# xdsopl/dwt

Measured on AMD Instinct MI355X. Metric: Mpixels/s lossless encode+decode round-trip, higher is better.
Workload: dtype int32; 1 GPU; 4096x4096x1 8-bit synthetic smooth+noise frames, lossless, 128 frames per GPU per step (BASELINE.json configs[1] geometry); frames_per_gpu=128, parallelism=1 GPU

## Files before the change

### dwt_amd/csrc/unpack.hip

```cpp
#include "hilbert_dev.h"

#include <stdlib.h>
#include <string.h>
#include <vector>

namespace {

constexpr int TILE = 1024;
constexpr int MAX_PLANES = 16;
constexpr int MAX_SEGS = 3 * 16 * MAX_PLANES;
constexpr int CH_LOG2 = 7;
constexpr int CH_BITS = 1 << CH_LOG2;
constexpr int SCAN_BLOCK = 1024;
constexpr int LINK_ROUNDS = 12;
constexpr int FAM = 2;

struct UnpackGeom {
	int levels, C, W, H;
	long total;
	long lin_stride;
	int pixels[DWTX_MAX_LEVELS + 1];
	int tile_first[DWTX_MAX_LEVELS + 1];
	int levels_max;
	int *pyr;
	short *fine16;
	unsigned lv16;
	unsigned sq_levels;
	int side[DWTX_MAX_LEVELS + 1];
	const int *tile_base;
	const unsigned short *tile_cnt;
	const int *tile_blk;
};

struct DecInfo {
	int status;
	int W, H, C;
	int levels;
	int planes[3];
	int pmax;
	int level;
	int nsegs;
	int truncated;
	int missing[48];
	unsigned long long bits_used;
	unsigned hops, hopped_chunks;
	unsigned walked_tokens;
	unsigned zeros_left;
};

struct SegIndex {
	unsigned long long bit;
	unsigned long long sym_base;
	unsigned n1;
	unsigned cnt;
	unsigned desc;
	unsigned order;
};

struct SegResult {
	unsigned long long bit;
	unsigned order, cnt, ones;
	unsigned nhops, hopped, walked;
	unsigned ok;
	unsigned pad;
};

struct DWork {
	DecInfo *info;
	int *seg_desc;
	unsigned long long *seg_symbase;
	unsigned long long *seg_b2;
	unsigned *seg_n2done;
	int *segidx;
	int *nonsig;
	unsigned *symbits;
	unsigned short *tile_nonsig;
	unsigned *tile_rank;
	unsigned long long *count_base;
	long BW;
	int NT;
	unsigned short *exitX;
	unsigned short *entryE;
	unsigned long long *cs;
	unsigned *ct;
	unsigned *cg;
	unsigned long long *part_s;
	unsigned *part_t, *part_g;
	int *hop_seg;
	unsigned *hop_first, *hop_last, *hop_q0;
	unsigned *hop_entry;
	unsigned *hop_ntok;
	unsigned *breaks;
	unsigned *todo[2];
	unsigned *todo_count;
	long todo_round;
	long todo_cap;
	unsigned long long *dbg;
	int *nhops;
	int *nch;
	long NCH, NB;
	long MAX_HOPS;
	SegIndex *idx;
	SegResult *segres;
	int *idx_nsegs;
	unsigned *seg_slot;
	int fam;
	unsigned streak_max, scans_base;
};

__device__ __forceinline__ int vstream(const DWork &w, int row) { return (row / w.fam) * FAM + row % w.fam; }

__device__ __forceinline__ int popc_below(unsigned long long m)
{
	return __builtin_amdgcn_mbcnt_hi((unsigned)(m >> 32), __builtin_amdgcn_mbcnt_lo((unsigned)m, 0));
}


struct BitReader {
	const unsigned long long *w;
	long n64;
	unsigned long long end_bits;
	unsigned long long b;
	unsigned long long base;
	unsigned long long f0, f1, f2, f3, f4, f5;

	__device__ __forceinline__ unsigned long long ld(unsigned long long bit) const
	{
		const long i = (long)(bit >> 6);
		return i < n64 ? w[i] : 0ull;
	}
	__device__ void seek(unsigned long long nb)
	{
		b = nb;
		base = nb & ~63ull;
		f0 = ld(base);
		f1 = ld(base + 64);
		f2 = ld(base + 128);
		f3 = ld(base + 192);
		f4 = ld(base + 256);
		f5 = ld(base + 320);
	}
	__device__ __forceinline__ unsigned long long peek()
	{
		while (b - base >= 64) {
			f0 = f1;
			f1 = f2;
			f2 = f3;
			f3 = f4;
			f4 = f5;
			base += 64;
			f5 = ld(base + 320);
		}
		const int off = (int)(b - base);
		return off ? (f0 >> off) | (f1 << (64 - off)) : f0;
	}
	__device__ __forceinline__ unsigned long long avail() const { return end_bits > b ? end_bits - b : 0ull; }
	__device__ __forceinline__ bool read(int n, unsigned &v)
	{
		if ((unsigned long long)n > avail())
			return false;
		const unsigned long long win = peek();
		v = n >= 32 ? (unsigned)win : (unsigned)win & ((1u << n) - 1u);
		b += n;
		return true;
	}
	__device__ __forceinline__ bool vli(int &order, unsigned &val)
	{
		const unsigned long long win = peek();
		const unsigned long long av = avail();
		const int z = win ? __builtin_ctzll(win) : 64;
		if ((unsigned long long)z >= av)
			return false;
		const int top = order + z;
		if (top > 31)
			return false;
		const int need = z + 1 + top;
		if ((unsigned long long)need > av)
			return false;
		const unsigned rem = top ? (unsigned)(win >> (z + 1)) & (unsigned)((1ull << top) - 1ull) : 0u;
		val = rem + (1u << top) - (1u << order);
		order = top >= 2 ? top - 2 : 0;
		b += need;
		return true;
	}
	__device__ bool read_any(unsigned n, unsigned &v)
	{
		if (n <= 32u)
			return read((int)n, v);
		unsigned a = 0;
		for (unsigned i = 0; i < n; ++i) {
			unsigned bit;
			if (!read(1, bit))
				return false;
			a |= bit << (i & 31u);
		}
		v = a;
		return true;
	}
	__device__ int vli_any(int &order, unsigned &val)
	{
		if (vli(order, val))
			return 0;
		unsigned ord = (unsigned)order, sum = 0;
		for (;;) {
			if (avail() >= 64 && !peek()) {
				sum += 2u * 0xffffffffu;
				ord += 64;
				b += 64;
				continue;
			}
			unsigned bit;
			if (!read(1, bit))
				return 1;
			if (bit)
				break;
			sum += 1u << (ord & 31u);
			++ord;
		}
		unsigned a = 0;
		for (unsigned i = 0; i < ord; ++i) {
			unsigned bit;
			if (!read(1, bit))
				return 1;
			a |= bit << (i & 31u);
		}
		order = ord >= 2u ? (int)(ord - 2u) : 0;
		const int v = (int)(a + sum);
		if (v < 0)
			return 2;
		val = (unsigned)v;
		return 0;
	}
};

struct BitmapWriter {
	unsigned *sym;
	long cur;
	unsigned acc;
	bool lead;
	__device__ __forceinline__ void flush()
	{
		if (cur >= 0 && acc && lead)
			atomicOr(sym + cur, acc);
		acc = 0;
	}
	__device__ __forceinline__ void set_one(unsigned long long pos)
	{
		const long wi = (long)(pos >> 4);
		if (wi != cur) {
			flush();
			cur = wi;
		}
		acc |= 1u << ((pos & 15) * 2);
	}
	__device__ __forceinline__ void set_sign(unsigned long long pos) { acc |= 2u << ((pos & 15) * 2); }
};


struct ChunkWin {
	unsigned long long w0, w1, w2;
};

__device__ __forceinline__ ChunkWin chunk_load(const unsigned long long *w64, long n64, long chunk)
{
	ChunkWin c;
	const long i = chunk * (CH_BITS / 64);
	c.w0 = i < n64 ? w64[i] : 0ull;
	c.w1 = i + 1 < n64 ? w64[i + 1] : 0ull;
	c.w2 = i + 2 < n64 ? w64[i + 2] : 0ull;
	return c;
}

__device__ __forceinline__ unsigned long long chunk_win(const ChunkWin &c, int off)
{
	const int r = off & 63;
	const unsigned long long lo = off >> 6 ? c.w1 : c.w0, hi = off >> 6 ? c.w2 : c.w1;
	return r ? (lo >> r) | (hi << (64 - r)) : lo;
}

__device__ __forceinline__ unsigned bfm(unsigned width, unsigned offset)
{
	unsigned r;
	asm("v_bfm_b32 %0, %1, %2" : "=v"(r) : "v"(width), "v"(offset));
	return r;
}

__device__ __forceinline__ bool token_at(unsigned long long win, int o, int &len, unsigned &run, unsigned &neg, int &next)
{
	if (!win)
		return false;
	const int z = __builtin_ctzll(win);
	const int top = o + z;
	if (top > 31)
		return false;
	len = z + top + 2;
	run = (top ? (unsigned)(win >> (z + 1)) & (unsigned)((1ull << top) - 1ull) : 0u) + (1u << top) - (1u << o);
	neg = (unsigned)(win >> (z + 1 + top)) & 1u;
	next = top >= 2 ? top - 2 : 0;
	return true;
}

#pragma clang diagnostic ignored "-Wpass-failed"
template <class F>
__device__ __forceinline__ bool chunk_walk(const ChunkWin &c, int &off, int &o, F &&visit)
{
	const unsigned d[6] = { (unsigned)c.w0, (unsigned)(c.w0 >> 32), (unsigned)c.w1, (unsigned)(c.w1 >> 32),
		(unsigned)c.w2, (unsigned)(c.w2 >> 32) };
	bool dead = false, stop = false;
#pragma unroll
	for (int seg = 0; seg < CH_BITS / 32; ++seg) {
		for (;;) {
			const int bound = 32 * (seg + 1);
			bool fits = !(stop || dead), go = true;
			while (off < bound && fits && go) {
				const unsigned w32 = __builtin_amdgcn_alignbit(d[seg + 1], d[seg], (unsigned)off);
				const int z = __builtin_ctz(w32 | 0x80000000u);
				const int top = o + z;
				const int len = z + top + 2;
				fits = len <= 32;
				const unsigned run = __builtin_amdgcn_ubfe(w32, (unsigned)(z + 1), (unsigned)top) + bfm((unsigned)z, (unsigned)o);
				const unsigned neg = __builtin_amdgcn_ubfe(w32, (unsigned)(len - 1), 1u);
				go = visit(run, neg, fits);
				const bool adv = fits && go;
				off += adv ? len : 0;
				o = adv ? (int)__builtin_elementwise_sub_sat((unsigned)top, 2u) : o;
			}
			stop = stop || !go;
			const bool slow = !fits && !stop && !dead;
			if (!ballot64(slow))
				break;
			if (slow) {
				const int r = off & 31;
				const unsigned long long lo64 = d[seg] | ((unsigned long long)d[seg + 1] << 32);
				const unsigned long long w64 = r ? (lo64 >> r) | ((unsigned long long)d[seg + 2] << (64 - r)) : lo64;
				int len, next;
				unsigned run, neg;
				if (!token_at(w64, o, len, run, neg, next)) {
					dead = true;
				} else if (visit(run, neg, true)) {
					off += len;
					o = next;
				} else {
					stop = true;
				}
			}
		}
	}
	return !dead;
}

template <class V, class K, class U>
__device__ __forceinline__ bool chunk_walk_all(const ChunkWin &c, int &off, int &o, V &&visit, K &&keep, U &&undo)
{
	const unsigned d[6] = { (unsigned)c.w0, (unsigned)(c.w0 >> 32), (unsigned)c.w1, (unsigned)(c.w1 >> 32),
		(unsigned)c.w2, (unsigned)(c.w2 >> 32) };
	bool dead = false;
#pragma unroll
	for (int seg = 0; seg < CH_BITS / 32; ++seg) {
		for (;;) {
			const int bound = 32 * (seg + 1);
			int len = 0, o_prev = o;
			while (off < bound) {
				o_prev = o;
				keep();
				const unsigned w32 = __builtin_amdgcn_alignbit(d[seg + 1], d[seg], (unsigned)off);
				const int z = __builtin_ctz(w32 | 0x80000000u);
				const int top = o + z;
				len = z + top + 2;
				visit(__builtin_amdgcn_ubfe(w32, (unsigned)(z + 1), (unsigned)top) + bfm((unsigned)z, (unsigned)o),
					__builtin_amdgcn_ubfe(w32, (unsigned)(len - 1), 1u), len <= 32);
				off += len;
				o = (int)__builtin_elementwise_sub_sat((unsigned)top, 2u);
			}
			const bool slow = len > 32;
			if (!ballot64(slow))
				break;
			if (slow) {
				off -= len;
				o = o_prev;
				undo();
				const int r = off & 31;
				const unsigned long long lo64 = d[seg] | ((unsigned long long)d[seg + 1] << 32);
				const unsigned long long w64 = r ? (lo64 >> r) | ((unsigned long long)d[seg + 2] << (64 - r)) : lo64;
				int len64, next;
				unsigned run, neg;
				if (!token_at(w64, o, len64, run, neg, next)) {
					dead = true;
					off = 2 * CH_BITS + 64;
				} else {
					visit(run, neg, true);
					off += len64;
					o = next;
				}
			}
		}
	}
	return !dead;
}

__device__ __forceinline__ bool chunk_count(const ChunkWin &c, int &off, int &o, unsigned &tok, unsigned &sym)
{
	unsigned sym_prev = sym;
	return chunk_walk_all(c, off, o,
		[&](unsigned run, unsigned, bool) {
			sym = __builtin_elementwise_add_sat(sym, run + 1u);
			++tok;
		},
		[&]() { sym_prev = sym; },
		[&]() {
			--tok;
			sym = sym_prev;
		});
}

__device__ __forceinline__ unsigned wave_incl_add_u(unsigned v)
{
	v += (unsigned)__builtin_amdgcn_update_dpp(0, (int)v, 0x111, 0xf, 0xf, false);
	v += (unsigned)__builtin_amdgcn_update_dpp(0, (int)v, 0x112, 0xf, 0xf, false);
	v += (unsigned)__builtin_amdgcn_update_dpp(0, (int)v, 0x114, 0xf, 0xf, false);
	v += (unsigned)__builtin_amdgcn_update_dpp(0, (int)v, 0x118, 0xf, 0xf, false);
	v += (unsigned)__builtin_amdgcn_update_dpp(0, (int)v, 0x142, 0xa, 0xf, false);
	v += (unsigned)__builtin_amdgcn_update_dpp(0, (int)v, 0x143, 0xc, 0xf, false);
	return v;
}

struct ChunkScan {
	unsigned tok, sym;
	int off, o;
	unsigned cross_run;
	int cross_bits, cross_o;
};

__device__ __forceinline__ ChunkScan chunk_scan(const ChunkWin &c, int off, int o, unsigned need)
{
	const int lane = (int)threadIdx.x & 63;
	const unsigned d0 = (unsigned)c.w0, d1 = (unsigned)(c.w0 >> 32), d2 = (unsigned)c.w1, d3 = (unsigned)(c.w1 >> 32),
		d4 = (unsigned)c.w2;
	const bool up = lane >= 32;
	const unsigned winA = __builtin_amdgcn_alignbit(up ? d2 : d1, up ? d1 : d0, (unsigned)lane & 31u);
	const unsigned winB = __builtin_amdgcn_alignbit(up ? d4 : d3, up ? d3 : d2, (unsigned)lane & 31u);
	{
		const int zA = winA ? __builtin_ctz(winA) : 32, zB = winB ? __builtin_ctz(winB) : 32;
		int ordA = -1, ordB = -1, offf = __builtin_amdgcn_readfirstlane(off), of2 = __builtin_amdgcn_readfirstlane(o) + 2;
		while (offf < 64) {
			const int z = __builtin_amdgcn_readlane(zA, offf);
			ordA = lane == offf ? of2 : ordA;
			const int top2 = of2 + z;
			offf += top2 + z;
			of2 = max(top2 - 2, 2);
		}
		while (offf < 128) {
			const int z = __builtin_amdgcn_readlane(zB, offf - 64);
			ordB = lane == offf - 64 ? of2 : ordB;
			const int top2 = of2 + z;
			offf += top2 + z;
			of2 = max(top2 - 2, 2);
		}
		const int of = of2 - 2;
		ordA = ordA < 0 ? -1 : ordA - 2;
		ordB = ordB < 0 ? -1 : ordB - 2;
		const bool longA = ordA >= 0 && 2 * zA + ordA > 30, longB = ordB >= 0 && 2 * zB + ordB > 30;
		const int worst = ballot64(longA || longB) ? 31 : 0;
		if (worst <= 30) {
			constexpr unsigned CAP = 1u << 24;
			auto cost = [&](unsigned win, int z, int ord) -> unsigned {
				const int top = ord + z;
				const unsigned run = ((win >> ((z + 1) & 31)) & ((1u << (top & 31)) - 1u)) + (1u << (top & 31)) - (1u << (ord & 31));
				return ord < 0 ? 0u : min(run + 1u, CAP);
			};
			const unsigned cA = cost(winA, zA, ordA), cB = cost(winB, zB, ordB);
			const unsigned long long visA = ballot64(ordA >= 0), visB = ballot64(ordB >= 0);
			const bool capped = ballot64(cA == CAP || cB == CAP) != 0;
			int v = (int)(cA + cB);
			v += __builtin_amdgcn_update_dpp(0, v, 0xB1, 0xf, 0xf, true);
			v += __builtin_amdgcn_update_dpp(0, v, 0x4E, 0xf, 0xf, true);
			v += __builtin_amdgcn_update_dpp(0, v, 0x141, 0xf, 0xf, true);
			v += __builtin_amdgcn_update_dpp(0, v, 0x140, 0xf, 0xf, true);
			const unsigned symf = (unsigned)(__builtin_amdgcn_readlane(v, 0) + __builtin_amdgcn_readlane(v, 16) +
				__builtin_amdgcn_readlane(v, 32) + __builtin_amdgcn_readlane(v, 48));
			if (!capped && symf <= need) {
				ChunkScan r = { (unsigned)(__builtin_popcountll(visA) + __builtin_popcountll(visB)), symf, offf, of, 0u, 0, 0 };
				return r;
			}
			if (!capped) {
				const unsigned need_s = (unsigned)__builtin_amdgcn_readfirstlane((int)need);
				const unsigned pA = wave_incl_add_u(cA);
				const unsigned totA = (unsigned)__builtin_amdgcn_readlane((int)pA, 63);
				const unsigned pB = totA + wave_incl_add_u(cB);
				const unsigned long long fitA = ballot64(ordA >= 0 && pA <= need_s), fitB = ballot64(ordB >= 0 && pB <= need_s);
				const unsigned long long restA = visA & ~fitA, restB = visB & ~fitB;
				unsigned sym = 0;
				if (fitB)
					sym = (unsigned)__builtin_amdgcn_readlane((int)pB, 63 - __builtin_clzll(fitB));
				else if (fitA)
					sym = (unsigned)__builtin_amdgcn_readlane((int)pA, 63 - __builtin_clzll(fitA));
				int off2, o2, z2;
				unsigned c2;
				if (restA) {
					const int at = __builtin_ctzll(restA);
					off2 = at;
					o2 = __builtin_amdgcn_readlane(ordA, at);
					z2 = __builtin_amdgcn_readlane(zA, at);
					c2 = (unsigned)__builtin_amdgcn_readlane((int)cA, at);
				} else {
					const int at = __builtin_ctzll(restB);
					off2 = 64 + at;
					o2 = __builtin_amdgcn_readlane(ordB, at);
					z2 = __builtin_amdgcn_readlane(zB, at);
					c2 = (unsigned)__builtin_amdgcn_readlane((int)cB, at);
				}
				const int top2 = o2 + z2;
				ChunkScan r = { (unsigned)(__builtin_popcountll(fitA) + __builtin_popcountll(fitB)), sym, off2, o2, c2 - 1u, z2 + top2 + 1, max(top2, 2) - 2 };
				return r;
			}
		}
	}
	const unsigned need_s = (unsigned)__builtin_amdgcn_readfirstlane((int)need);
	unsigned tok = 0, left = need_s;
	off = __builtin_amdgcn_readfirstlane(off);
	o = __builtin_amdgcn_readfirstlane(o);
	auto token = [&](unsigned w32) -> bool {
		const int z = w32 ? __builtin_ctz(w32) : 32;
		const int top = o + z;
		const unsigned run = ((w32 >> ((z + 1) & 31)) & ((1u << (top & 31)) - 1u)) + (1u << (top & 31)) - (1u << o);
		const bool ok = z + top <= 30 && run < left;
		left -= ok ? run + 1u : 0u;
		tok += ok ? 1u : 0u;
		off += ok ? z + top + 2 : 0;
		o = ok ? max(top, 2) - 2 : o;
		return ok;
	};
	bool ok = true;
	while (ok && off < 64)
		ok = token((unsigned)__builtin_amdgcn_readlane((int)winA, off));
	while (ok && off < 128)
		ok = token((unsigned)__builtin_amdgcn_readlane((int)winB, off - 64));
	ChunkScan r = { tok, need_s - left, off, o, 0u, 0, 0 };
	return r;
}

constexpr int CHUNK_GRID = 2048;

constexpr int LINK_SHARDS = 64;
constexpr int LINK_RUN = 8;
constexpr int RUN_W = 2 * LINK_RUN + 2;

__device__ __forceinline__ bool link_parse(const DWork &w, const unsigned char *streams, long stream_stride, int vs, long ch)
{
	const int img = vs / FAM;
	const long ci = vs * (w.NCH + 1) + ch;
	const unsigned short in = w.exitX[vs * w.NCH + ch - 1];
	unsigned sym = 0, tok = 0;
	unsigned short out = 0xffff;
	if (in != 0xffff) {
		const ChunkWin c = chunk_load((const unsigned long long *)(streams + img * stream_stride), stream_stride >> 3, ch);
		int off = in & 0xff, o = in >> 8;
		if (chunk_count(c, off, o, tok, sym))
			out = (unsigned short)((off - CH_BITS) | (o << 8));
	}
	const unsigned short old = w.exitX[vs * w.NCH + ch];
	w.entryE[vs * w.NCH + ch] = in;
	w.cs[ci] = sym;
	w.ct[ci] = tok;
	w.exitX[vs * w.NCH + ch] = out;
	return out != old && ch + 1 < w.nch[img];
}

__device__ __forceinline__ void link_push(const DWork &w, int vs, long ch, bool want, unsigned *next_list, unsigned *next_count)
{
	const int lane = threadIdx.x & 63;
	const int shard = (int)((ch >> 8) % LINK_SHARDS);
	unsigned long long todo = ballot64(want);
	while (todo) {
		const int leader = __builtin_ctzll(todo);
		const int sh = __shfl(shard, leader);
		const unsigned long long same = ballot64(want && shard == sh) & todo;
		unsigned base = 0;
		if (lane == leader)
			base = atomicAdd(next_count + vs * LINK_SHARDS + sh, (unsigned)__builtin_popcountll(same));
		base = __shfl(base, leader);
		if (want && shard == sh)
			next_list[((long)vs * LINK_SHARDS + sh) * w.todo_cap + base +
				(unsigned)__builtin_popcountll(same & ((1ull << lane) - 1ull))] = (unsigned)ch;
		todo &= ~same;
	}
}

__device__ __forceinline__ unsigned link_state13(unsigned short s) { return s == 0xffff ? 0x1fffu : ((unsigned)s & 0x7fu) | ((unsigned)s >> 8) << 7; }
__device__ __forceinline__ unsigned short link_state16(unsigned s) { return s == 0x1fffu ? (unsigned short)0xffff : (unsigned short)((s & 0x7fu) | (s >> 7) << 8); }
__device__ __forceinline__ unsigned long long link_record(unsigned sym, unsigned tok, unsigned short in, unsigned short out)
{
	const unsigned long long s31 = sym < 0x7fffffffu ? sym : 0x7fffffffu;
	return s31 | (unsigned long long)tok << 31 | (unsigned long long)link_state13(in) << 38 | (unsigned long long)link_state13(out) << 51;
}


__global__ __launch_bounds__(256) __attribute__((amdgpu_num_sgpr(64), amdgpu_waves_per_eu(4))) void k_link_first(DWork w, const unsigned char *streams, long stream_stride)
{
	__shared__ unsigned long long words[256 * RUN_W + 4];
	__shared__ unsigned short sx[256];
	const int vs = vstream(w, blockIdx.y), img = vs / FAM;
	const long nch = w.nch[img];
	const unsigned short start = (unsigned short)((w.fam == 1 ? 0 : CH_BITS / 2) + vs % FAM);
	const unsigned long long *w64 = (const unsigned long long *)(streams + img * stream_stride);
	const long n64 = stream_stride >> 3;
	constexpr long SPAN = 256 * LINK_RUN;
	for (long base = (long)blockIdx.x * SPAN; base < nch; base += (long)gridDim.x * SPAN) {
		const long g0 = 2 * (base - 1);
#pragma unroll
		for (int k = 0; k < (2 * (int)SPAN + 3 + 255) / 256; ++k) {
			const int L = k * 256 + (int)threadIdx.x;
			const long gi = g0 + L;
			if (L < 2 * (int)SPAN + 3)
				words[L + (L / (2 * LINK_RUN)) * 2] = gi >= 0 && gi < n64 ? w64[gi] : 0ull;
		}
		__syncthreads();
		const long c0 = base + (long)threadIdx.x * LINK_RUN;
		unsigned long long *mine = words + threadIdx.x * RUN_W;
		auto word = [&](int i) { return mine[i + (i >= 2 * LINK_RUN ? 2 : 0)]; };
		unsigned short st = start, wexit = 0xffff;
		unsigned long long carry = word(0);
		for (int j = 0; j <= LINK_RUN; ++j) {
			const long chunk = c0 - 1 + j;
			ChunkWin c = { carry, word(2 * j + 1), word(2 * j + 2) };
			carry = c.w2;
			unsigned long long rec = ~0ull;
			if (chunk >= 0 && chunk < nch) {
				const unsigned short in = j == 0 || chunk == 0 || st == 0xffff ? start : st;
				int off = in & 0xff, o = in >> 8;
				unsigned sym = 0, tok = 0;
				const bool alive = chunk_count(c, off, o, tok, sym);
				st = alive ? (unsigned short)((off - CH_BITS) | (o << 8)) : (unsigned short)0xffff;
				rec = link_record(sym, tok, in, st);
			}
			if (j == 0)
				wexit = st;
			else
				mine[2 + j] = rec;
		}
		sx[threadIdx.x] = st;
		__syncthreads();
#pragma unroll
		for (int k = 0; k < LINK_RUN; ++k) {
			const int q = k * 256 + (int)threadIdx.x;
			const long chunk = base + q;
			const unsigned long long rec = words[(q / LINK_RUN) * RUN_W + 3 + q % LINK_RUN];
			if (rec != ~0ull) {
				if (chunk > 0) {
					w.entryE[vs * w.NCH + chunk] = link_state16((unsigned)(rec >> 38) & 0x1fffu);
					w.cs[vs * (w.NCH + 1) + chunk] = rec & 0x7fffffffull;
					w.ct[vs * (w.NCH + 1) + chunk] = (unsigned)(rec >> 31) & 0x7fu;
				}
				w.exitX[vs * w.NCH + chunk] = link_state16((unsigned)(rec >> 51));
			}
		}
		const bool redo = c0 > 0 && c0 < nch && (threadIdx.x == 0 || sx[threadIdx.x - 1] != wexit);
		link_push(w, vs, c0, redo, w.todo[1], w.todo_count + 2 * w.todo_round);
		__syncthreads();
	}
}

__global__ __launch_bounds__(256) __attribute__((amdgpu_num_sgpr(64))) void k_link_work(DWork w, const unsigned char *streams, long stream_stride, int cur, int round)
{
	const int vs = vstream(w, blockIdx.y), shard = blockIdx.x % LINK_SHARDS, part = blockIdx.x / LINK_SHARDS,
		parts = gridDim.x / LINK_SHARDS;
	const unsigned count = w.todo_count[round * w.todo_round + vs * LINK_SHARDS + shard];
	const unsigned *list = w.todo[cur] + ((long)vs * LINK_SHARDS + shard) * w.todo_cap;
	for (unsigned q0 = part * blockDim.x; q0 < count; q0 += parts * blockDim.x) {
		const unsigned q = q0 + threadIdx.x;
		bool moved = false;
		long ch = 0;
		if (q < count) {
			ch = list[q];
			moved = link_parse(w, streams, stream_stride, vs, ch);
		}
		link_push(w, vs, ch + 1, moved, w.todo[cur ^ 1], w.todo_count + (round + 1) * w.todo_round);
	}
}

struct Tri {
	unsigned long long s;
	unsigned t, g;
};

__device__ __forceinline__ Tri tri_add(Tri a, Tri b)
{
	Tri r = { a.s + b.s, a.t + b.t, a.g + b.g };
	return r;
}

__device__ __forceinline__ Tri tri_shfl_up(Tri v, int o)
{
	Tri r;
	r.s = __shfl_up(v.s, o);
	r.t = __shfl_up(v.t, o);
	r.g = __shfl_up(v.g, o);
	return r;
}

__device__ __forceinline__ Tri block_scan_tri(Tri v, Tri *wsum, Tri &total)
{
	const int lane = threadIdx.x & 63, wv = threadIdx.x >> 6;
	Tri inc = v;
	for (int o = 1; o < 64; o <<= 1) {
		const Tri t = tri_shfl_up(inc, o);
		if (lane >= o)
			inc = tri_add(inc, t);
	}
	if (lane == 63)
		wsum[wv] = inc;
	__syncthreads();
	Tri off = { 0, 0, 0 }, all = { 0, 0, 0 };
	for (int k = 0; k < 4; ++k) {
		if (k < wv)
			off = tri_add(off, wsum[k]);
		all = tri_add(all, wsum[k]);
	}
	__syncthreads();
	total = all;
	Tri ex = { off.s + inc.s - v.s, off.t + inc.t - v.t, off.g + inc.g - v.g };
	return ex;
}

struct Quad {
	ulonglong2 s01, s23;
	uint4 t, g;
};

__device__ __forceinline__ Quad quad_load(const DWork &w, long at)
{
	Quad q;
	q.s01 = *reinterpret_cast<const ulonglong2 *>(w.cs + at);
	q.s23 = *reinterpret_cast<const ulonglong2 *>(w.cs + at + 2);
	q.t = *reinterpret_cast<const uint4 *>(w.ct + at);
	q.g = *reinterpret_cast<const uint4 *>(w.cg + at);
	return q;
}

__device__ __forceinline__ void quad_store(const DWork &w, long at, const Quad &q)
{
	*reinterpret_cast<ulonglong2 *>(w.cs + at) = q.s01;
	*reinterpret_cast<ulonglong2 *>(w.cs + at + 2) = q.s23;
	*reinterpret_cast<uint4 *>(w.ct + at) = q.t;
	*reinterpret_cast<uint4 *>(w.cg + at) = q.g;
}

constexpr int SCAN_GRID = 1024;

__global__ __launch_bounds__(256) void k_scan_local(DWork w)
{
	__shared__ Tri wsum[4];
	const int vs = vstream(w, blockIdx.y);
	const long n = w.NCH + 1, nch = w.nch[vs / FAM], used = nch + 1;
	unsigned short *exitX = w.exitX + (long)vs * w.NCH, *entryE = w.entryE + (long)vs * w.NCH;
	for (long vb = blockIdx.x; vb * SCAN_BLOCK < used; vb += gridDim.x) {
		const long i = vb * SCAN_BLOCK + 4 * threadIdx.x;
		const bool in = i < used;
		Quad q;
		q.s01 = q.s23 = make_ulonglong2(0ull, 0ull);
		q.t = q.g = make_uint4(0u, 0u, 0u, 0u);
		if (in) {
			q = quad_load(w, vs * n + i);
			unsigned long long *sv[4] = { &q.s01.x, &q.s01.y, &q.s23.x, &q.s23.y };
			unsigned *tv[4] = { &q.t.x, &q.t.y, &q.t.z, &q.t.w }, *gv[4] = { &q.g.x, &q.g.y, &q.g.z, &q.g.w };
			unsigned short prev = i >= 1 && i - 1 < nch ? exitX[i - 1] : (unsigned short)0xffff;
#pragma unroll
			for (int e = 0; e < 4; ++e) {
				const long c = i + e;
				unsigned flag;
				if (c == 0 || c >= nch) {
					flag = c == 0 ? 1u : 0u;
					*sv[e] = 0;
					*tv[e] = 0;
				} else {
					const unsigned short x = exitX[c];
					const bool bad = prev == 0xffff || entryE[c] != prev || x == 0xffff;
					flag = bad ? 1u : 0u;
					if (bad) {
						*sv[e] = 0;
						*tv[e] = 0;
					}
					prev = x;
				}
				if (c == 0)
					prev = nch > 0 ? exitX[0] : (unsigned short)0xffff;
				*gv[e] = flag;
				if (c < nch)
					entryE[c] = (unsigned short)flag;
			}
		}
		const Tri mine = { q.s01.x + q.s01.y + q.s23.x + q.s23.y, q.t.x + q.t.y + q.t.z + q.t.w, q.g.x + q.g.y + q.g.z + q.g.w };
		Tri total;
		const Tri pre = block_scan_tri(mine, wsum, total);
		if (in) {
			Quad o;
			o.s01.x = pre.s;
			o.s01.y = o.s01.x + q.s01.x;
			o.s23.x = o.s01.y + q.s01.y;
			o.s23.y = o.s23.x + q.s23.x;
			o.t.x = pre.t;
			o.t.y = o.t.x + q.t.x;
			o.t.z = o.t.y + q.t.y;
			o.t.w = o.t.z + q.t.z;
			o.g.x = pre.g;
			o.g.y = o.g.x + q.g.x;
			o.g.z = o.g.y + q.g.y;
			o.g.w = o.g.z + q.g.z;
			quad_store(w, vs * n + i, o);
		}
		if (threadIdx.x == 0) {
			w.part_s[vs * w.NB + vb] = total.s;
			w.part_t[vs * w.NB + vb] = total.t;
			w.part_g[vs * w.NB + vb] = total.g;
		}
		__syncthreads();
	}
}

__global__ __launch_bounds__(256) void k_scan_parts(DWork w)
{
	__shared__ Tri wsum[4];
	const int img = vstream(w, blockIdx.x);
	const long nb = (w.nch[img / FAM] + 1 + SCAN_BLOCK - 1) / SCAN_BLOCK;
	Tri carry = { 0, 0, 0 };
	for (long b0 = 0; b0 < nb; b0 += 256) {
		const long i = b0 + threadIdx.x;
		Tri v = { 0, 0, 0 };
		if (i < nb) {
			v.s = w.part_s[img * w.NB + i];
			v.t = w.part_t[img * w.NB + i];
			v.g = w.part_g[img * w.NB + i];
		}
		Tri total;
		const Tri pre = block_scan_tri(v, wsum, total);
		if (i < nb) {
			w.part_s[img * w.NB + i] = carry.s + pre.s;
			w.part_t[img * w.NB + i] = carry.t + pre.t;
			w.part_g[img * w.NB + i] = carry.g + pre.g;
		}
		carry = tri_add(carry, total);
	}
}

__global__ __launch_bounds__(256) void k_scan_add(DWork w)
{
	const int vs = vstream(w, blockIdx.y);
	const long n = w.NCH + 1, nch = w.nch[vs / FAM], used = nch + 1;
	const unsigned short *flags = w.entryE + (long)vs * w.NCH;
	unsigned *breaks = w.breaks + (long)vs * w.NCH;
	for (long vb = blockIdx.x; vb * SCAN_BLOCK < used; vb += gridDim.x) {
		const long i = vb * SCAN_BLOCK + 4 * threadIdx.x;
		if (i >= used)
			continue;
		const unsigned long long ps = w.part_s[vs * w.NB + vb];
		const unsigned pt = w.part_t[vs * w.NB + vb], pg = w.part_g[vs * w.NB + vb];
		Quad q = quad_load(w, vs * n + i);
		q.s01.x += ps;
		q.s01.y += ps;
		q.s23.x += ps;
		q.s23.y += ps;
		q.t.x += pt;
		q.t.y += pt;
		q.t.z += pt;
		q.t.w += pt;
		q.g.x += pg;
		q.g.y += pg;
		q.g.z += pg;
		q.g.w += pg;
		if (vb)
			quad_store(w, vs * n + i, q);
		const unsigned g4[4] = { q.g.x, q.g.y, q.g.z, q.g.w };
#pragma unroll
		for (int e = 0; e < 4; ++e)
			if (i + e < nch && flags[i + e])
				breaks[g4[e]] = (unsigned)(i + e);
	}
}

__global__ __launch_bounds__(256) __attribute__((amdgpu_waves_per_eu(8))) void k_hopbits(DWork w, const unsigned char *streams, long stream_stride)
{
	constexpr int HB_WORDS = 16;
	constexpr int HB_WIN = 2048;
	__shared__ unsigned hb[256 * (HB_WORDS + 1)];
	static_assert(HB_WIN <= 256 * (HB_WORDS + 1), "the workgroup's window lies inside the per-thread rows");
	unsigned *win = hb;
	__shared__ unsigned win_last;
	for (int i = 0; i <= HB_WORDS; ++i)
		hb[threadIdx.x * (HB_WORDS + 1) + i] = 0u;
	const int img = blockIdx.y;
	const int nh = w.nhops[img];
	const long nchunks = w.nch[img];
	const unsigned *hf = w.hop_first + (long)img * w.MAX_HOPS, *hl = w.hop_last + (long)img * w.MAX_HOPS;
	for (long vblock = blockIdx.x; vblock * blockDim.x < nchunks; vblock += gridDim.x) {
	const long chunk = vblock * blockDim.x + threadIdx.x;
	const unsigned first_chunk = (unsigned)(vblock * blockDim.x);
	int lo = 0, hi = nh;
	while (lo < hi) {
		const int mid = (lo + hi) >> 1;
		if (hl[mid] < first_chunk)
			lo = mid + 1;
		else
			hi = mid;
	}
	unsigned *sym = w.symbits + img * w.BW;
	const long n = w.NCH + 1;
	ChunkWin c;
	bool loaded = false;
	unsigned *mybuf = hb + threadIdx.x * (HB_WORDS + 1);
	auto piece = [&](int h) {
		const int hs = w.hop_seg[(long)img * w.MAX_HOPS + h];
		const int k = hs & 0xffff, vs = img * FAM + (hs >> 16);
		if ((w.seg_desc[(long)img * MAX_SEGS + k] >> 8) == 0)
			return;
		if (!loaded) {
			c = chunk_load((const unsigned long long *)(streams + img * stream_stride), stream_stride >> 3, chunk);
			loaded = true;
		}
		unsigned long long pos = w.seg_symbase[(long)img * MAX_SEGS + k] + w.hop_q0[(long)img * w.MAX_HOPS + h];
		const unsigned entry = w.hop_entry[(long)img * w.MAX_HOPS + h];
		unsigned left = w.hop_ntok[(long)img * w.MAX_HOPS + h];
		int off, o;
		if (entry == 0xffffffffu) {
			pos += w.cs[vs * n + chunk] - w.cs[vs * n + hf[h]];
			const unsigned short in = w.exitX[vs * w.NCH + chunk - 1];
			off = in & 0xff;
			o = in >> 8;
		} else {
			off = (int)(entry & 0xff);
			o = (int)(entry >> 8);
		}
		unsigned *wp = sym + (pos >> 4);
		const unsigned rp0 = (unsigned)(pos & 15);
		unsigned rp = rp0;
		bool beyond = false;
		const int off0 = off, o0 = o;
		chunk_walk(c, off, o, [&](unsigned run, unsigned neg, bool counts) {
			const bool take = counts && left != 0u;
			rp += take ? run : 0u;
			const unsigned wi = rp >> 4;
			beyond = beyond || (take && wi >= (unsigned)HB_WORDS);
			atomicOr(&mybuf[wi < (unsigned)HB_WORDS ? wi : (unsigned)HB_WORDS], take ? (1u | (neg << 1)) << ((rp & 15u) * 2u) : 0u);
			rp += take ? 1u : 0u;
			left -= take ? 1u : 0u;
			return left != 0u || !counts;
		});
		if (beyond) {
			unsigned rq = rp0, lq = w.hop_ntok[(long)img * w.MAX_HOPS + h];
			int off1 = off0, o1 = o0;
			chunk_walk(c, off1, o1, [&](unsigned run, unsigned neg, bool counts) {
				const bool take = counts && lq != 0u;
				rq += take ? run : 0u;
				if (take && (rq >> 4) >= (unsigned)HB_WORDS)
					atomicOr(wp + (rq >> 4), (1u | (neg << 1)) << ((rq & 15u) * 2u));
				rq += take ? 1u : 0u;
				lq -= take ? 1u : 0u;
				return lq != 0u || !counts;
			});
			mybuf[HB_WORDS] = 0u;
		}
		const unsigned lastw = rp > rp0 ? (rp - 1) >> 4 : 0u;
#pragma unroll
		for (int i = 0; i < HB_WORDS; ++i) {
			const unsigned v = mybuf[i];
			if (v) {
				if (i == 0 || (unsigned)i >= lastw)
					atomicOr(wp + i, v);
				else
					wp[i] = v;
				mybuf[i] = 0u;
			}
		}
	};
	const bool mine = chunk < w.nch[img] && chunk >= 1;
	if (lo < nh && hf[lo] <= first_chunk && hl[lo] >= first_chunk + blockDim.x - 1 && (lo + 1 >= nh || hf[lo + 1] > first_chunk + blockDim.x - 1)) {
		const int hs = w.hop_seg[(long)img * w.MAX_HOPS + lo];
		const int k = hs & 0xffff, vs = img * FAM + (hs >> 16);
		const bool stitched = w.hop_entry[(long)img * w.MAX_HOPS + lo] == 0xffffffffu && first_chunk >= 1;
		if (!stitched) {
			if (mine)
				piece(lo);
			continue;
		}
		if ((w.seg_desc[(long)img * MAX_SEGS + k] >> 8) == 0)
			continue;
		const unsigned long long seg0 = w.seg_symbase[(long)img * MAX_SEGS + k] + w.hop_q0[(long)img * w.MAX_HOPS + lo] -
			w.cs[vs * n + hf[lo]];
		const unsigned long long base_w = (seg0 + w.cs[vs * n + first_chunk]) >> 4;
		if (threadIdx.x == 0)
			win_last = 0u;
		__syncthreads();
		{
			const ChunkWin cw = chunk_load((const unsigned long long *)(streams + img * stream_stride), stream_stride >> 3, chunk);
			const unsigned short in = w.exitX[vs * w.NCH + chunk - 1];
			int off = in & 0xff, o = in >> 8;
			unsigned roff = (unsigned)(seg0 + w.cs[vs * n + chunk] - (base_w << 4));
			const unsigned roff0 = roff;
			unsigned *gp = sym + base_w;
			unsigned roff_prev = roff;
			chunk_walk_all(cw, off, o,
				[&](unsigned run, unsigned neg, bool fits) {
					roff += run;
					const unsigned wi = roff >> 4;
					const unsigned bits = fits ? (1u | (neg << 1)) << ((roff & 15u) * 2u) : 0u;
					if (wi < (unsigned)HB_WIN)
						atomicOr(&win[wi], bits);
					else if (fits)
						atomicOr(gp + wi, bits);
					++roff;
				},
				[&]() { roff_prev = roff; }, [&]() { roff = roff_prev; });
			if (roff > roff0) {
				const unsigned lw = (roff - 1) >> 4;
				atomicMax(&win_last, lw < (unsigned)HB_WIN - 1u ? lw : (unsigned)HB_WIN - 1u);
			}
		}
		__syncthreads();
		{
			const unsigned lastw = win_last;
			unsigned *gp = sym + base_w;
			for (unsigned i = threadIdx.x; i <= lastw; i += 256) {
				const unsigned v = win[i];
				win[i] = 0u;
				if (i > 0 && i < lastw)
					gp[i] = v;
				else if (v)
					atomicOr(gp + i, v);
			}
		}
		__syncthreads();
		continue;
	}
	if (!mine)
		continue;
	int h = lo;
	while (h < nh && hl[h] < (unsigned)chunk)
		++h;
	for (; h < nh && hf[h] <= (unsigned)chunk; ++h)
		piece(h);
	}
}

__global__ __launch_bounds__(256) void k_part_reset(DWork h, int cnt)
{
	const long t = (long)blockIdx.x * blockDim.x + threadIdx.x;
	const long per_round = (long)cnt * FAM * LINK_SHARDS;
	if (t < per_round)
		for (int r = 0; r < LINK_ROUNDS + 2; ++r)
			h.todo_count[r * h.todo_round + t] = 0u;
	if (t < cnt)
		h.nhops[t] = 0;
	if (t < (long)cnt * 48 * MAX_PLANES)
		h.segidx[t] = 0;
	if (t < (long)cnt * (long)(sizeof(DecInfo) / sizeof(int)))
		reinterpret_cast<int *>(h.info)[t] = 0;
}

__device__ int read_preamble(BitReader &br, const UnpackGeom &g, const unsigned char *s8, unsigned long long len, long stream_stride,
	int &order, int (&planes)[3], int *root, long root_stride)
{
	if (len < 6 || s8[0] != 'W' || s8[1] != (g.C == 3 ? '6' : '5') ||
		(s8[2] | (s8[3] << 8)) + 1 != g.W || (s8[4] | (s8[5] << 8)) + 1 != g.H)
		return 1;
	br.w = (const unsigned long long *)s8;
	br.n64 = stream_stride >> 3;
	br.end_bits = len * 8;
	br.seek(48);
	order = 0;
	for (int c = 0; c < g.C; ++c) {
		unsigned cnt;
		if (br.vli_any(order, cnt))
			return 1;
		if (cnt)
			for (int i = 0; i < g.pixels[0]; ++i) {
				unsigned v, neg = 0;
				if (!br.read_any(cnt, v))
					return 1;
				if (v && !br.read(1, neg))
					return 1;
				if (root)
					root[c * root_stride + i] = neg ? -(int)v : (int)v;
			}
	}
	for (int c = 0; c < g.C; ++c) {
		unsigned p;
		if (br.vli_any(order, p))
			return 1;
		if (p > MAX_PLANES)
			return 2;
		planes[c] = (int)p;
	}
	return 0;
}

__global__ __launch_bounds__(64) void k_peek(UnpackGeom g, const unsigned char *streams, long stream_stride, const unsigned long long *lens,
	long BW, unsigned *clear_words, int n)
{
	const int img = blockIdx.x * blockDim.x + threadIdx.x;
	if (img >= n)
		return;
	const unsigned char *s8 = streams + img * stream_stride;
	const unsigned long long len = lens[img] < (unsigned long long)stream_stride ? lens[img] : (unsigned long long)stream_stride;
	BitReader br;
	int order, planes[3] = { 0, 0, 0 };
	unsigned long long words = 0;
	if (!read_preamble(br, g, s8, len, stream_stride, order, planes, nullptr, 0)) {
		unsigned long long per = 0;
		for (int l = 0; l < g.levels; ++l)
			per += ((unsigned long long)(g.pixels[l + 1] - g.pixels[l]) + 31) & ~31ull;
		unsigned long long sym = ((unsigned long long)(g.pixels[1] - g.pixels[0]) + 31) & ~31ull;
		for (int c = 0; c < g.C; ++c)
			sym += (unsigned long long)planes[c] * per;
		words = ((sym >> 4) + 128 + 3) & ~3ull;
	}
	clear_words[img] = (unsigned)(words < (unsigned long long)BW ? words : (unsigned long long)BW);
}

__global__ __launch_bounds__(256) void k_clear_bitmaps(unsigned *bits, long BW, const unsigned *clear_words)
{
	uint4 *dst = reinterpret_cast<uint4 *>(bits + (long)blockIdx.y * BW);
	const unsigned quads = clear_words[blockIdx.y] >> 2;
	for (unsigned i = blockIdx.x * blockDim.x + threadIdx.x; i < quads; i += gridDim.x * blockDim.x)
		dst[i] = make_uint4(0u, 0u, 0u, 0u);
}


template <class F, class M>
__device__ __forceinline__ bool walk_schedule(const UnpackGeom &g, const int (&planes)[3], int pmax, int &level, M &&one_less_missing, F &&seg)
{
	const int levels = g.levels;
	const int layers_max = 2 * (levels > pmax ? levels : pmax) - 1;
	bool stop = g.levels_max == 0;
	if (!stop && pmax == planes[0]) {
		level = 0;
		if (seg(0, 0, planes[0] - 1))
			one_less_missing(0);
		else
			stop = true;
	}
	for (int layer = 0; !stop && layer < layers_max; ++layer) {
		for (int l = 0; !stop && l < levels && l <= layer + 1; ++l) {
			if (l >= g.levels_max) {
				stop = true;
				break;
			}
			const int p = pmax - 1 - (layer + 1 - l);
			if (p < 0 || p >= planes[0])
				continue;
			level = level < l ? l : level;
			if (seg(0, l, p))
				one_less_missing(l);
			else
				stop = true;
		}
		for (int l = 0; !stop && l < levels && l <= layer; ++l) {
			if (l >= g.levels_max) {
				stop = true;
				break;
			}
			const int p = pmax - 1 - (layer - l);
			for (int c = 1; !stop && c < g.C; ++c) {
				if (p < 0 || p >= planes[c])
					continue;
				level = level < l ? l : level;
				if (seg(c, l, p))
					one_less_missing(c * 16 + l);
				else
					stop = true;
			}
		}
	}
	return stop;
}

constexpr unsigned WALK_STREAK_MAX = 256u, WALK_SCANS_BASE = 256u;
constexpr unsigned WALK_GAVE_UP = 0xffffffffu;

__device__ __forceinline__ void info_begin(DecInfo &I, const UnpackGeom &g)
{
	I.status = 1;
	I.W = g.W;
	I.H = g.H;
	I.C = g.C;
	I.levels = g.levels;
	I.level = -1;
	I.nsegs = 0;
	I.truncated = 0;
	I.pmax = 0;
	for (int i = 0; i < 48; ++i)
		I.missing[i] = 0;
}

template <bool SEG>
__global__ __launch_bounds__(64) void k_tokenize(UnpackGeom g, DWork w, const unsigned char *streams, long stream_stride,
	const unsigned long long *lens, int *lin, int n)
{
	const int img = SEG ? blockIdx.y : blockIdx.x;
	if (img >= n)
		return;
	const int seg_k = SEG ? (int)blockIdx.x : 0;
	if (SEG && seg_k >= w.idx_nsegs[img])
		return;
	DecInfo &I = w.info[img];
	const unsigned char *s8 = streams + img * stream_stride;
	const unsigned long long len = lens[img] < (unsigned long long)stream_stride ? lens[img] : (unsigned long long)stream_stride;
	BitReader br;
	int order = 0;
	int planes[3] = { 0, 0, 0 };
	int pmax = 0;
	int nonsig_own[1] = { 0 };
	int nonsig_v = 0;
	SegIndex *idx = w.idx + (long)img * MAX_SEGS;
	if (!SEG) {
		info_begin(I, g);
		if (const int bad = read_preamble(br, g, s8, len, stream_stride, order, planes, lin + (long)img * g.C * g.lin_stride, g.lin_stride)) {
			I.status = bad;
			return;
		}
		for (int c = 0; c < g.C; ++c) {
			I.planes[c] = planes[c];
			pmax = planes[c] > pmax ? planes[c] : pmax;
		}
		I.pmax = pmax;
		I.status = 0;
		for (int c = 0; c < g.C; ++c)
			for (int l = 0; l < g.levels; ++l)
				I.missing[c * 16 + l] = planes[c];
		{
			const int lv = (int)threadIdx.x & 15, ch = (int)threadIdx.x >> 4;
			nonsig_v = ch < g.C && lv < g.levels ? g.pixels[lv + 1] - g.pixels[lv] : 0;
		}
	} else {
		br.w = (const unsigned long long *)s8;
		br.n64 = stream_stride >> 3;
		br.end_bits = len * 8;
		br.b = idx[seg_k].bit < br.end_bits ? idx[seg_k].bit : br.end_bits;
		br.base = 0;
		br.f0 = br.f1 = br.f2 = br.f3 = br.f4 = br.f5 = 0;
		order = (int)(idx[seg_k].order & 31u);
		nonsig_own[0] = (int)idx[seg_k].n1;
	}
	int *sd = w.seg_desc + (long)img * MAX_SEGS;
	unsigned long long *ssym = w.seg_symbase + (long)img * MAX_SEGS;
	unsigned long long *sb2 = w.seg_b2 + (long)img * MAX_SEGS;
	unsigned *sn2 = w.seg_n2done + (long)img * MAX_SEGS;
	int *sidx = w.segidx + (long)img * 3 * 16 * MAX_PLANES;
	BitmapWriter bm;
	bm.sym = w.symbits + img * w.BW;
	bm.cur = -1;
	bm.acc = 0;
	bm.lead = threadIdx.x == 0;
	const int wl = (int)threadIdx.x;

	unsigned cnt = SEG ? idx[seg_k].cnt : 0u;
	unsigned long long symtotal = SEG ? idx[seg_k].sym_base : 0ull;
	int nsegs = seg_k, level = -1;

	const unsigned short *exitX0 = w.exitX + (long)img * FAM * w.NCH;
	const unsigned long long *CS0 = w.cs + (long)img * FAM * (w.NCH + 1);
	const unsigned *CT0 = w.ct + (long)img * FAM * (w.NCH + 1), *CG0 = w.cg + (long)img * FAM * (w.NCH + 1);
	const unsigned *BR0 = w.breaks + (long)img * FAM * w.NCH;
	const unsigned long long *s64 = (const unsigned long long *)s8;
	const long lastsafe = br.end_bits >= 64 + CH_BITS ? (long)((br.end_bits - 64) >> CH_LOG2) - 1 : -1;
#ifdef DWTX_DEBUG_HOOKS
	unsigned long long t_hop = 0, t_fast = 0, t_load = 0, t_scan = 0, t_care = 0, n_care = 0, t_all0 = __builtin_readcyclecounter(), t_mark = 0;
#define WALK_MARK() t_mark = __builtin_readcyclecounter()
#define WALK_ADD(acc) do { const unsigned long long t_now = __builtin_readcyclecounter(); acc += t_now - t_mark; t_mark = t_now; } while (0)
#else
#define WALK_MARK()
#define WALK_ADD(acc)
#endif
	unsigned scans = 0, streak = 0;
	bool giveup = false;
	long checked = -1;
	int nhops = 0;
	unsigned hopped = 0, walked = 0;
	bool br_synced = !SEG;
	bool eof = false;
	const long hop0 = (long)img * w.MAX_HOPS + (SEG ? (long)w.seg_slot[(long)img * (MAX_SEGS + 1) + seg_k] : 0l);
	const long hop_cap = SEG ? (long)(w.seg_slot[(long)img * (MAX_SEGS + 1) + seg_k + 1] - w.seg_slot[(long)img * (MAX_SEGS + 1) + seg_k]) : w.MAX_HOPS;
	int *hop_seg = w.hop_seg + hop0;
	unsigned *hop_first = w.hop_first + hop0, *hop_last = w.hop_last + hop0, *hop_q0 = w.hop_q0 + hop0, *hop_entry = w.hop_entry + hop0,
		*hop_ntok = w.hop_ntok + hop0;

	auto segment = [&](int c, int l, int p) -> bool {
		const int num = g.pixels[l + 1] - g.pixels[l];
		const int n1 = p < 0 ? num : SEG ? nonsig_own[0] : __builtin_amdgcn_readlane(nonsig_v, c * 16 + l);
		const int n2 = num - n1;
		const int k = nsegs++;
		const unsigned long long sym0 = symtotal;
		if (!SEG) {
			SegIndex e;
			e.bit = br.b;
			e.sym_base = sym0;
			e.n1 = (unsigned)n1;
			e.cnt = cnt;
			e.desc = (unsigned)(c | (l << 4) | ((p + 1) << 8));
			e.order = (unsigned)order;
			idx[k] = e;
		}
		symtotal += ((unsigned long long)num + 31) & ~31ull;
		sd[k] = c | (l << 4) | ((p + 1) << 8);
		ssym[k] = sym0;
		sb2[k] = 0;
		sn2[k] = 0;
		if (p >= 0)
			sidx[(c * 16 + l) * MAX_PLANES + p] = k + 1;
		int q = 0, ones = 0;
		bool ok = true;
		streak = 0;
		while (q < n1) {
			unsigned zr;
			if (cnt == 0) {
				const long ci = (long)(br.b >> CH_LOG2);
				if (ci >= 1 && ci <= lastsafe && nhops < hop_cap) {
					const unsigned need = (unsigned)(n1 - q);
					const int rel = (int)(br.b - ((unsigned long long)ci << CH_LOG2));
					bool moved = false;
					WALK_MARK();
					if (ci != checked) {
						checked = ci;
						for (int fam = 0; fam < w.fam && !moved; ++fam) {
							const unsigned ep = exitX0[fam * w.NCH + ci - 1];
							if (ep == 0xffffu || (int)(ep & 0xffu) != rel || (int)(ep >> 8) != order)
								continue;
							const unsigned long long *CS = CS0 + fam * (w.NCH + 1);
							const unsigned *CT = CT0 + fam * (w.NCH + 1), *CG = CG0 + fam * (w.NCH + 1);
							const unsigned g0 = CG[ci], g1 = CG[ci + 1], gtot = CG[w.nch[img]];
							if (g1 != g0)
								continue;
							const unsigned long long s0 = CS[ci];
							long hi = g0 < gtot ? (long)BR0[fam * w.NCH + g0] - 1 : lastsafe;
							hi = hi < lastsafe ? hi : lastsafe;
							long lo = ci - 1;
							if (hi >= ci && CS[hi + 1] - s0 <= (unsigned long long)need) {
								lo = hi;
							} else {
								hi = hi - 1;
								while (lo < hi) {
									const long span = hi - lo, stride = (span + 63) >> 6;
									const long step = (long)(wl + 1) * stride;
									const long probe = lo + (step < span ? step : span);
									const int t = __builtin_popcountll(ballot64(CS[probe + 1] - s0 <= (unsigned long long)need));
									const long reach = (long)t * stride, next = (long)(t + 1) * stride;
									hi = t == 64 ? hi : lo + (next < span ? next : span) - 1;
									lo = lo + (reach < span ? reach : span);
								}
							}
							if (lo >= ci) {
								hop_seg[nhops] = k | (fam << 16);
								hop_first[nhops] = (unsigned)ci;
								hop_last[nhops] = (unsigned)lo;
								hop_q0[nhops] = (unsigned)q;
								hop_entry[nhops] = 0xffffffffu;
								hop_ntok[nhops] = 0xffffffffu;
								++nhops;
								hopped += (unsigned)(lo - ci + 1);
								q += (int)(CS[lo + 1] - s0);
								ones += (int)(CT[lo + 1] - CT[ci]);
								const unsigned eq = exitX0[fam * w.NCH + lo];
								order = (int)(eq >> 8);
								br.b = ((unsigned long long)(lo + 1) << CH_LOG2) + (eq & 0xffu);
								br_synced = false;
								moved = true;
							}
						}
					}
					WALK_ADD(t_hop);
					if (moved)
						streak = 0;
					if (!moved) {
						++scans;
						++streak;
						if (w.fam < FAM && (streak > w.streak_max || scans > w.scans_base + 16u * (unsigned)nsegs + (unsigned)(lastsafe >> 9))) {
							giveup = true;
							return false;
						}
						const ChunkWin cwv = chunk_load(s64, br.n64, ci);
#ifdef DWTX_DEBUG_HOOKS
						asm volatile("s_waitcnt vmcnt(0) lgkmcnt(0)" ::: "memory");
						WALK_ADD(t_load);
#endif
						const ChunkScan cs = chunk_scan(cwv, rel, order, need);
#ifdef DWTX_DEBUG_HOOKS
						WALK_ADD(t_scan);
#endif
						const unsigned tok = cs.tok, sym = cs.sym;
						const int off = cs.off, o = cs.o;
						if (tok) {
							hop_seg[nhops] = k;
							hop_first[nhops] = (unsigned)ci;
							hop_last[nhops] = (unsigned)ci;
							hop_q0[nhops] = (unsigned)q;
							hop_entry[nhops] = (unsigned)rel | ((unsigned)order << 8);
							hop_ntok[nhops] = tok;
							++nhops;
							walked += tok;
							q += (int)sym;
							ones += (int)tok;
							order = o;
							br.b = ((unsigned long long)ci << CH_LOG2) + (unsigned)off;
							br_synced = false;
							moved = true;
						}
						if (cs.cross_bits && q < n1) {
							const unsigned rem = (unsigned)(n1 - q);
							++walked;
							order = cs.cross_o;
							br.b = ((unsigned long long)ci << CH_LOG2) + (unsigned)off + (unsigned)cs.cross_bits;
							br_synced = false;
							q = n1;
							cnt = cs.cross_run - rem + 1;
							WALK_ADD(t_fast);
							break;
						}
					}
					WALK_ADD(t_fast);
					if (moved)
						continue;
				}
#ifdef DWTX_DEBUG_HOOKS
				WALK_MARK();
				++n_care;
#endif
				if (!br_synced) {
					br.seek(br.b);
					br_synced = true;
				}
				unsigned v;
				const int bad = br.vli_any(order, v);
				if (bad) {
					ok = false;
					eof = bad == 1;
					break;
				}
				++walked;
				zr = v;
#ifdef DWTX_DEBUG_HOOKS
				WALK_ADD(t_care);
#endif
			} else {
				zr = cnt - 1;
			}
			const unsigned rem = (unsigned)(n1 - q);
			if (zr >= rem) {
				q = n1;
				cnt = zr - rem + 1;
				break;
			}
			q += (int)zr;
			cnt = 0;
			if (p >= 0)
				bm.set_one(sym0 + (unsigned)q);
			++ones;
			if (!br_synced) {
				br.seek(br.b);
				br_synced = true;
			}
			unsigned neg;
			if (!br.read(1, neg)) {
				++q;
				ok = false;
				eof = true;
				break;
			}
			if (neg && p >= 0)
				bm.set_sign(sym0 + (unsigned)q);
			++q;
		}
		if (p >= 0) {
			if (SEG)
				nonsig_own[0] = n1 - ones;
			else
				nonsig_v = wl == c * 16 + l ? n1 - ones : nonsig_v;
		}
		if (!ok)
			return false;
		if (p >= 0 && n2 > 0) {
			if (cnt > 0) {
				if (cnt != 1) {
					--cnt;
					return false;
				}
				cnt = 0;
			}
			sb2[k] = br.b;
			const unsigned long long av = br.avail();
			if ((unsigned long long)n2 > av) {
				sn2[k] = (unsigned)av;
				br.b = br.end_bits;
				eof = true;
				return false;
			}
			sn2[k] = (unsigned)n2;
			br.b += (unsigned)n2;
			br_synced = false;
		}
		return true;
	};

	bool stop = false;
	if (SEG) {
		const unsigned d = idx[seg_k].desc;
		const int c = (int)(d & 15u), l = (int)((d >> 4) & 15u), p = (int)(d >> 8) - 1;
		const unsigned long long ring = (unsigned long long)(g.pixels[l < g.levels ? l + 1 : 1] - g.pixels[l < g.levels ? l : 0]);
		const unsigned long long sym_cap = (unsigned long long)w.BW * 16ull;
		const bool sane = c < g.C && l < g.levels && p < MAX_PLANES && (unsigned long long)idx[seg_k].n1 <= ring && idx[seg_k].order <= 31u &&
			ring + 32ull <= sym_cap && idx[seg_k].sym_base <= sym_cap - ring - 32ull;
		const bool went = sane && segment(c, l, p);
		bm.flush();
		SegResult r;
		r.bit = br.b;
		r.order = (unsigned)order;
		r.cnt = cnt;
		r.ones = sane ? idx[seg_k].n1 - (unsigned)nonsig_own[0] : 0u;
		r.nhops = (unsigned)nhops;
		r.hopped = hopped;
		r.walked = walked;
		r.ok = went && !giveup && !eof ? 1u : 0u;
		r.pad = 0u;
		w.segres[(long)img * MAX_SEGS + seg_k] = r;
		return;
	}
	int missing_v = wl < 48 && (wl >> 4) < g.C && (wl & 15) < g.levels ? planes[wl >> 4 < 3 ? wl >> 4 : 0] : 0;
	stop = walk_schedule(g, planes, pmax, level, [&](int i) { missing_v = wl == i ? missing_v - 1 : missing_v; }, segment);
	if (wl < 48 && (wl >> 4) < g.C && (wl & 15) < g.levels)
		I.missing[wl] = missing_v;
	bm.flush();
	if (giveup) {
		w.nhops[img] = 0;
		I.hops = WALK_GAVE_UP;
		return;
	}
	w.nhops[img] = nhops;
	I.hops = (unsigned)nhops;
	I.hopped_chunks = hopped;
	I.walked_tokens = walked;
	I.zeros_left = cnt;
#ifdef DWTX_DEBUG_HOOKS
	if (w.dbg) { w.dbg[img * 8 + 0] = __builtin_readcyclecounter() - t_all0; w.dbg[img * 8 + 1] = t_hop; w.dbg[img * 8 + 2] = t_fast; w.dbg[img * 8 + 3] = scans;
		w.dbg[img * 8 + 4] = t_load; w.dbg[img * 8 + 5] = t_scan; w.dbg[img * 8 + 6] = t_care; w.dbg[img * 8 + 7] = n_care; }
#endif
	I.level = level;
	I.nsegs = nsegs;
	I.truncated = stop ? (eof ? 3 : 1) : 0;
	I.bits_used = br.b;
}

__global__ __launch_bounds__(64) void k_segprep(DWork w, const unsigned long long *lens, long stream_stride, int n)
{
	const int img = blockIdx.x * blockDim.x + threadIdx.x;
	if (img >= n)
		return;
	const int K = w.idx_nsegs[img];
	const SegIndex *idx = w.idx + (long)img * MAX_SEGS;
	unsigned *slot = w.seg_slot + (long)img * (MAX_SEGS + 1);
	const unsigned long long end_bits = 8ull * (lens[img] < (unsigned long long)stream_stride ? lens[img] : (unsigned long long)stream_stride);
	bool good = K > 0 && K <= MAX_SEGS;
	unsigned long long at = 0;
	for (int k = 0; good && k < K; ++k) {
		const unsigned long long b = idx[k].bit, nb = k + 1 < K ? idx[k + 1].bit : end_bits;
		good = b <= nb && nb <= end_bits && idx[k].sym_base < (unsigned long long)w.BW * 16ull && idx[k].order <= 31u;
		slot[k] = (unsigned)at;
		at += 8ull + ((nb - b) >> (CH_LOG2 + 3));
	}
	slot[K > 0 && K <= MAX_SEGS ? K : 0] = (unsigned)at;
	if (!good || at > (unsigned long long)w.MAX_HOPS)
		w.idx_nsegs[img] = 0;
}

__global__ __launch_bounds__(64) void k_segjoin(UnpackGeom g, DWork w, const unsigned char *streams, long stream_stride,
	const unsigned long long *lens, int *lin, int n)
{
	const int img = blockIdx.x;
	if (img >= n)
		return;
	const int lane = threadIdx.x;
	DecInfo &I = w.info[img];
	info_begin(I, g);
	const unsigned char *s8 = streams + img * stream_stride;
	const unsigned long long len = lens[img] < (unsigned long long)stream_stride ? lens[img] : (unsigned long long)stream_stride;
	BitReader br;
	int order = 0, planes[3] = { 0, 0, 0 };
	if (const int bad = read_preamble(br, g, s8, len, stream_stride, order, planes, lin + (long)img * g.C * g.lin_stride, g.lin_stride)) {
		I.status = bad;
		return;
	}
	int pmax = 0;
	for (int c = 0; c < g.C; ++c) {
		I.planes[c] = planes[c];
		pmax = planes[c] > pmax ? planes[c] : pmax;
	}
	I.pmax = pmax;
	I.status = 0;
	for (int c = 0; c < g.C; ++c)
		for (int l = 0; l < g.levels; ++l)
			I.missing[c * 16 + l] = planes[c];
	const int K = w.idx_nsegs[img];
	const SegIndex *idx = w.idx + (long)img * MAX_SEGS;
	const SegResult *res = w.segres + (long)img * MAX_SEGS;
	int nonsig[48];
	for (int c = 0; c < g.C; ++c)
		for (int l = 0; l < g.levels; ++l)
			nonsig[c * 16 + l] = g.pixels[l + 1] - g.pixels[l];
	unsigned long long at = br.b, symtotal = 0;
	unsigned cnt = 0, hopped = 0, walked = 0;
	int k = 0, level = -1;
	bool good = K > 0 && g.levels_max >= g.levels;
	const bool stop = walk_schedule(g, planes, pmax, level, [&](int i) { --I.missing[i]; }, [&](int c, int l, int p) {
		const int num = g.pixels[l + 1] - g.pixels[l];
		const int n1 = p < 0 ? num : nonsig[c * 16 + l];
		good = good && k < K;
		if (good) {
			const SegIndex e = idx[k];
			const SegResult r = res[k];
			good = e.desc == (unsigned)(c | (l << 4) | ((p + 1) << 8)) && e.bit == at && e.order == (unsigned)order && e.cnt == cnt &&
				e.n1 == (unsigned)n1 && e.sym_base == symtotal && r.ok != 0u && r.ones <= (unsigned)n1;
			if (good) {
				at = r.bit;
				order = (int)r.order;
				cnt = r.cnt;
				if (p >= 0)
					nonsig[c * 16 + l] = n1 - (int)r.ones;
				symtotal += ((unsigned long long)num + 31) & ~31ull;
				hopped += r.hopped;
				walked += r.walked;
				++k;
			}
		}
		return good;
	});
	good = good && !stop && k == K;
	if (!good) {
		w.nhops[img] = 0;
		I.hops = WALK_GAVE_UP;
		return;
	}
	const unsigned *slot = w.seg_slot + (long)img * (MAX_SEGS + 1);
	const long h0 = (long)img * w.MAX_HOPS;
	unsigned total = 0;
	for (int j = 0; j < K; ++j) {
		const unsigned nh = res[j].nhops, from = slot[j];
		if (from != total)
			for (unsigned i0 = 0; i0 < nh; i0 += 64) {
				const unsigned i = i0 + (unsigned)lane;
				int a = 0;
				unsigned b = 0, c2 = 0, d = 0, e = 0, f = 0;
				if (i < nh) {
					a = w.hop_seg[h0 + from + i];
					b = w.hop_first[h0 + from + i];
					c2 = w.hop_last[h0 + from + i];
					d = w.hop_q0[h0 + from + i];
					e = w.hop_entry[h0 + from + i];
					f = w.hop_ntok[h0 + from + i];
				}
				if (i < nh) {
					w.hop_seg[h0 + total + i] = a;
					w.hop_first[h0 + total + i] = b;
					w.hop_last[h0 + total + i] = c2;
					w.hop_q0[h0 + total + i] = d;
					w.hop_entry[h0 + total + i] = e;
					w.hop_ntok[h0 + total + i] = f;
				}
			}
		total += nh;
	}
	w.nhops[img] = (int)total;
	I.hops = total;
	I.hopped_chunks = hopped;
	I.walked_tokens = walked;
	I.zeros_left = cnt;
	I.level = level;
	I.nsegs = K;
	I.truncated = 0;
	I.bits_used = at;
}


__global__ __launch_bounds__(1024) void k_rank(UnpackGeom g, DWork w, int p)
{
	__shared__ unsigned wsum[16];
	__shared__ unsigned carry;
	const int l = blockIdx.x;
	const int plane = blockIdx.y;
	const int img = plane / g.C, c = plane - img * g.C;
	const int k1 = w.info[img].status ? 0 : w.segidx[((long)img * 48 + c * 16 + l) * MAX_PLANES + p];
	if (threadIdx.x == 0)
		w.count_base[(long)plane * 16 + l] = k1 ? 1ull + 2ull * w.seg_symbase[(long)img * MAX_SEGS + k1 - 1] : 0ull;
	if (!k1)
		return;
	const int t0 = g.tile_first[l], nt = g.tile_first[l + 1] - t0;
	const unsigned short *ns = w.tile_nonsig + (long)plane * w.NT + t0;
	unsigned *rank = w.tile_rank + ((long)plane * MAX_PLANES + p) * w.NT + t0;
	const int lane = threadIdx.x & 63, wv = threadIdx.x >> 6;
	if (threadIdx.x == 0)
		carry = 0;
	__syncthreads();
	for (int b0 = 0; b0 < nt; b0 += 1024) {
		const int i = b0 + threadIdx.x;
		const unsigned v = i < nt ? ns[i] : 0u;
		unsigned inc = v;
		for (int o = 1; o < 64; o <<= 1) {
			const unsigned t = __shfl_up(inc, o);
			if (lane >= o)
				inc += t;
		}
		if (lane == 63)
			wsum[wv] = inc;
		__syncthreads();
		unsigned woff = 0, all = 0;
		for (int k = 0; k < 16; ++k) {
			const unsigned s = wsum[k];
			woff += k < wv ? s : 0u;
			all += s;
		}
		const unsigned cy = carry;
		if (i < nt)
			rank[i] = cy + woff + inc - v;
		__syncthreads();
		if (threadIdx.x == 0)
			carry = cy + all;
		__syncthreads();
	}
}

__global__ __launch_bounds__(256) void k_count(UnpackGeom g, DWork w, int p)
{
	const int tile = blockIdx.x * blockDim.x + threadIdx.x;
	const int plane = blockIdx.y;
	const int img = plane / g.C;
	if (tile >= w.NT)
		return;
	int l = 0;
	while (l + 1 < g.levels && tile >= g.tile_first[l + 1])
		++l;
	const unsigned long long cb = w.count_base[(long)plane * 16 + l];
	if (!cb)
		return;
	unsigned short *ns = w.tile_nonsig + (long)plane * w.NT + tile;
	unsigned *rk = w.tile_rank + ((long)plane * MAX_PLANES + p) * w.NT + tile;
	const unsigned n = *ns;
	if (!n)
		return;
	const unsigned *sym = w.symbits + img * w.BW;
	const unsigned long long a = cb - 1ull + 2ull * *rk;
	const unsigned long long e = a + 2ull * n;
	const long first = (long)(a >> 5), last = (long)((e - 1) >> 5);
	unsigned ones = 0;
#pragma unroll 4
	for (long w0 = first & ~3l; w0 <= last; w0 += 4) {
		const uint4 v = *reinterpret_cast<const uint4 *>(sym + w0);
		const unsigned x[4] = { v.x, v.y, v.z, v.w };
#pragma unroll
		for (int q = 0; q < 4; ++q) {
			const long wi = w0 + q;
			unsigned m = x[q] & 0x55555555u;
			if (wi < first || wi > last)
				m = 0u;
			if (wi == first)
				m &= ~0u << (a & 31);
			if (wi == last && (e & 31))
				m &= (1u << (e & 31)) - 1u;
			ones += (unsigned)__builtin_popcount(m);
		}
	}
	if (ones) {
		*ns = (unsigned short)(n - ones);
		*rk |= 0x80000000u;
	}
}

__device__ __forceinline__ void bit_transpose8(unsigned &lo, unsigned &hi)
{
	unsigned t;
	t = (lo ^ (lo >> 7)) & 0x00AA00AAu;
	lo ^= t ^ (t << 7);
	t = (hi ^ (hi >> 7)) & 0x00AA00AAu;
	hi ^= t ^ (t << 7);
	t = (lo ^ (lo >> 14)) & 0x0000CCCCu;
	lo ^= t ^ (t << 14);
	t = (hi ^ (hi >> 14)) & 0x0000CCCCu;
	hi ^= t ^ (t << 14);
	const unsigned nlo = (lo & 0x0F0F0F0Fu) | ((hi << 4) & 0xF0F0F0F0u);
	hi = ((lo >> 4) & 0x0F0F0F0Fu) | (hi & 0xF0F0F0F0u);
	lo = nlo;
}

struct DepositTables {
	unsigned char sym[16 * 256];
	unsigned char ref[16 * 16];
};

constexpr DepositTables make_deposit_tables()
{
	DepositTables t{};
	for (unsigned m = 0; m < 16; ++m) {
		for (unsigned s = 0; s < 256; ++s) {
			unsigned ones = 0, signs = 0, k = 0;
			for (unsigned j = 0; j < 4; ++j)
				if ((m >> j) & 1u) {
					const unsigned one = (s >> (2 * k)) & 1u, sg = (s >> (2 * k + 1)) & 1u;
					ones |= one << j;
					signs |= (one & sg) << j;
					++k;
				}
			t.sym[m * 256 + s] = (unsigned char)(ones | signs << 4);
		}
		for (unsigned b = 0; b < 16; ++b) {
			unsigned out = 0, k = 0;
			for (unsigned j = 0; j < 4; ++j)
				if ((m >> j) & 1u) {
					out |= ((b >> k) & 1u) << j;
					++k;
				}
			t.ref[m * 16 + b] = (unsigned char)out;
		}
	}
	return t;
}

__device__ const DepositTables DEPOSIT = make_deposit_tables();

struct __attribute__((packed, aligned(4))) Int4S {
	int x, y, z, w;
};

__global__ __launch_bounds__(256) __attribute__((amdgpu_waves_per_eu(6))) void k_apply_all(UnpackGeom g, DWork w, const unsigned char *streams, long stream_stride, int *lin)
{
	__shared__ __attribute__((aligned(16))) unsigned char dep[sizeof(DepositTables)];
	static_assert(sizeof(DepositTables) == 17 * 256, "one 16-byte piece and one byte per thread");
	*reinterpret_cast<uint4 *>(dep + 16 * threadIdx.x) = *reinterpret_cast<const uint4 *>(DEPOSIT.sym + 16 * threadIdx.x);
	dep[4096 + threadIdx.x] = DEPOSIT.ref[threadIdx.x];
	__syncthreads();
	const unsigned char *dsym = dep, *dref = dep + 4096;
	const int lane = threadIdx.x & 63;
	const int tile = blockIdx.x * 4 + (threadIdx.x >> 6);
	const int plane = blockIdx.y;
	if (tile >= w.NT)
		return;
	const int img = plane / g.C, c = plane - img * g.C;
	const DecInfo &I = w.info[img];
	if (I.status)
		return;
	int l = 0;
	while (l + 1 < g.levels && tile >= g.tile_first[l + 1])
		++l;
	const unsigned tbase = (unsigned)g.tile_base[tile];
	const long base = g.pixels[l] + (long)tbase;
	const int nvalid = g.tile_cnt[tile];
	const int first = 16 * lane;
	const int nv = nvalid - first < 0 ? 0 : nvalid - first > 16 ? 16 : nvalid - first;
	const int vb = first < nvalid ? first : nvalid;
	const unsigned *sym = w.symbits + img * w.BW;
	const unsigned *stream = (const unsigned *)(streams + img * stream_stride);
	const long stream_words = stream_stride >> 2;
	unsigned R[8] = { 0u, 0u, 0u, 0u, 0u, 0u, 0u, 0u };
	int p_last = 0, rows_in = 0;
	auto push_row = [&](unsigned row16) {
		if (rows_in >= 8) {
#pragma unroll
			for (int k = 7; k >= 4; --k)
				R[k] = __builtin_amdgcn_alignbit(R[k], R[k - 1], 16);
		}
		if (rows_in >= 6)
			R[3] = __builtin_amdgcn_alignbit(R[3], R[2], 16);
		if (rows_in >= 4)
			R[2] = __builtin_amdgcn_alignbit(R[2], R[1], 16);
		if (rows_in >= 2)
			R[1] = __builtin_amdgcn_alignbit(R[1], R[0], 16);
		R[0] = (R[0] << 16) | row16;
		++rows_in;
	};
	unsigned neg = 0;
	const unsigned valid16 = nv >= 16 ? 0xffffu : (1u << nv) - 1u;
	unsigned ins = valid16;

	constexpr int AP_BATCH = 8, SYMW = 66, REFW = 34;
	static_assert(AP_BATCH * (SYMW + REFW) <= SQ_WORDS, "the plane slices share the wave's square staging area");
	__shared__ __attribute__((aligned(16))) unsigned ap_mem[4][SQ_WORDS];
	unsigned (*ap_sym)[SYMW] = reinterpret_cast<unsigned (*)[SYMW]>(ap_mem[threadIdx.x >> 6]);
	unsigned (*ap_ref)[REFW] = reinterpret_cast<unsigned (*)[REFW]>(ap_mem[threadIdx.x >> 6] + AP_BATCH * SYMW);
	__shared__ unsigned ap_rank[4][MAX_PLANES], ap_n2[4][MAX_PLANES], ap_refbit[4][MAX_PLANES];
	const int wv = threadIdx.x >> 6;
	unsigned my_tr = 0, my_n2 = 0;
	unsigned long long my_sb = 0, my_b2 = 0;
	bool my_live = false;
	if (lane < MAX_PLANES && lane < I.planes[c]) {
		const int k1 = w.segidx[((long)img * 48 + c * 16 + l) * MAX_PLANES + lane];
		if (k1) {
			my_live = true;
			my_tr = w.tile_rank[((long)plane * MAX_PLANES + lane) * w.NT + tile];
			my_sb = w.seg_symbase[(long)img * MAX_SEGS + k1 - 1];
			my_b2 = w.seg_b2[(long)img * MAX_SEGS + k1 - 1];
			my_n2 = w.seg_n2done[(long)img * MAX_SEGS + k1 - 1];
		}
	}
	const unsigned long long livem = ballot64(my_live), flagm = ballot64(my_live && (my_tr >> 31));
	const int ptop = flagm ? 63 - __builtin_clzll(flagm) : -1;
	unsigned long long todo = ptop >= 0 ? livem & ((2ull << ptop) - 1ull) : 0ull;
	while (todo) {
		int pl[AP_BATCH];
		unsigned long long t2 = todo;
#pragma unroll
		for (int q = 0; q < AP_BATCH; ++q) {
			pl[q] = t2 ? 63 - __builtin_clzll(t2) : -1;
			t2 &= pl[q] >= 0 ? ~(1ull << pl[q]) : ~0ull;
		}
		unsigned sv0[AP_BATCH], sv1[AP_BATCH], rv[AP_BATCH];
#pragma unroll
		for (int q = 0; q < AP_BATCH; ++q) {
			sv0[q] = sv1[q] = rv[q] = 0u;
			if (pl[q] < 0)
				continue;
			const unsigned rank = (unsigned)__builtin_amdgcn_readlane((int)my_tr, pl[q]) & 0x7fffffffu;
			const unsigned long long sb = ((unsigned long long)(unsigned)__builtin_amdgcn_readlane((int)(my_sb >> 32), pl[q]) << 32) |
				(unsigned)__builtin_amdgcn_readlane((int)my_sb, pl[q]);
			const unsigned long long b2 = ((unsigned long long)(unsigned)__builtin_amdgcn_readlane((int)(my_b2 >> 32), pl[q]) << 32) |
				(unsigned)__builtin_amdgcn_readlane((int)my_b2, pl[q]);
			const unsigned n2 = (unsigned)__builtin_amdgcn_readlane((int)my_n2, pl[q]);
			const unsigned *sp = sym + (sb >> 4) + (rank >> 4);
			sv0[q] = sp[lane];
			if (lane < SYMW - 64)
				sv1[q] = sp[64 + lane];
			const unsigned r2t = tbase - rank;
			const unsigned long long rbit = b2 + r2t;
			const long rw = (long)(rbit >> 5) + lane;
			if (lane < REFW && r2t < n2 && rw < stream_words)
				rv[q] = stream[rw];
			if (lane == 0) {
				ap_rank[wv][pl[q]] = rank;
				ap_n2[wv][pl[q]] = n2;
				ap_refbit[wv][pl[q]] = (unsigned)(rbit & 31);
			}
		}
#pragma unroll
		for (int q = 0; q < AP_BATCH; ++q) {
			if (pl[q] < 0)
				continue;
			ap_sym[q][lane] = sv0[q];
			if (lane < SYMW - 64)
				ap_sym[q][64 + lane] = sv1[q];
			if (lane < REFW)
				ap_ref[q][lane] = rv[q];
		}
		sq_wave_sync();
		const int nbatch = __builtin_popcountll(todo) < AP_BATCH ? __builtin_popcountll(todo) : AP_BATCH;
#pragma unroll 1
		for (int q = 0; q < nbatch; ++q) {
			const int p = 63 - __builtin_clzll(todo);
			todo &= ~(1ull << p);
			const unsigned rank = ap_rank[wv][p], n2done = ap_n2[wv][p];
			const unsigned ci = (unsigned)__builtin_popcount(ins);
			const unsigned nb = wave_incl_add_u(ci) - ci;
			const unsigned srel = (rank & 15u) + nb;
			const unsigned *sw = ap_sym[q] + (srel >> 4);
			unsigned s32 = __builtin_amdgcn_alignbit(sw[1], sw[0], (srel & 15u) * 2u);
			const unsigned sb4 = (unsigned)vb - nb;
			const unsigned r2 = tbase - rank + sb4;
			const unsigned cs = (unsigned)nv - ci;
			const unsigned avail = r2 < n2done ? (n2done - r2 < cs ? n2done - r2 : cs) : 0u;
			const unsigned rrel = ap_refbit[wv][p] + sb4;
			const unsigned *rwp = ap_ref[q] + (rrel >> 5);
			unsigned r16 = __builtin_amdgcn_alignbit(rwp[1], rwp[0], rrel & 31u) & bfm(avail, 0u);
			const unsigned sig = valid16 & ~ins;
			unsigned ones16 = 0, sgn16 = 0, ref16 = 0;
#pragma unroll
			for (int n4 = 0; n4 < 4; ++n4) {
				const unsigned mi = (ins >> (4 * n4)) & 15u, ms = (sig >> (4 * n4)) & 15u;
				const unsigned es = dsym[mi * 256u + (s32 & 255u)], er = dref[ms * 16u + (r16 & 15u)];
				ones16 |= (es & 15u) << (4 * n4);
				sgn16 |= (es >> 4) << (4 * n4);
				ref16 |= er << (4 * n4);
				s32 >>= 2 * __builtin_popcount(mi);
				r16 >>= __builtin_popcount(ms);
			}
			const unsigned bits16 = ones16 | ref16;
			neg |= sgn16;
			ins &= ~ones16;
			for (int gap = rows_in ? p_last - p - 1 : 0; gap > 0; --gap)
				push_row(0u);
			push_row(bits16);
			p_last = p;
		}
		sq_wave_sync();
	}
	unsigned mag[16];
	{
		unsigned lo[2], hi[2];
#pragma unroll
		for (int gg = 0; gg < 2; ++gg) {
			const unsigned sel = (unsigned)gg * 0x01010101u + 0x06040200u;
			lo[gg] = __builtin_amdgcn_perm(R[1], R[0], sel);
			hi[gg] = __builtin_amdgcn_perm(R[3], R[2], sel);
			bit_transpose8(lo[gg], hi[gg]);
		}
#pragma unroll
		for (int i = 0; i < 16; ++i)
			mag[i] = __builtin_amdgcn_ubfe((i & 4) ? hi[i >> 3] : lo[i >> 3], 8u * (i & 3), 8u);
		if (rows_in > 8) {
#pragma unroll
			for (int gg = 0; gg < 2; ++gg) {
				const unsigned sel = (unsigned)gg * 0x01010101u + 0x06040200u;
				lo[gg] = __builtin_amdgcn_perm(R[5], R[4], sel);
				hi[gg] = __builtin_amdgcn_perm(R[7], R[6], sel);
				bit_transpose8(lo[gg], hi[gg]);
			}
#pragma unroll
			for (int i = 0; i < 16; ++i)
				mag[i] |= __builtin_amdgcn_ubfe((i & 4) ? hi[i >> 3] : lo[i >> 3], 8u * (i & 3), 8u) << 8;
		}
#pragma unroll
		for (int i = 0; i < 16; ++i)
			mag[i] <<= p_last;
	}
	if (((g.sq_levels >> l) & 1u) && nvalid == TILE) {
		const int m = I.missing[c * 16 + l] - 2;
		const int bias = m >= 0 ? 1 << m : 0;
		int val[16];
#pragma unroll
		for (int i = 0; i < 16; ++i) {
			int v = ((neg >> i) & 1u) ? -(int)mag[i] : (int)mag[i];
			if (bias && v)
				v += v < 0 ? -bias : bias;
			val[i] = v;
		}
		if ((g.lv16 >> l) & 1u)
			store_square16(g.fine16 + (long)plane * g.lin_stride, g.W, g.side[l], g.tile_blk[tile], lane, ap_mem[threadIdx.x >> 6], val);
		else
			store_square16(g.pyr + (long)plane * g.lin_stride, g.W, g.side[l], g.tile_blk[tile], lane, ap_mem[threadIdx.x >> 6], val);
		return;
	}
	int *dst = lin + (long)plane * g.lin_stride + base + first;
	if (nvalid == TILE) {
#pragma unroll
		for (int q = 0; q < 4; ++q) {
			Int4S v;
			v.x = ((neg >> (4 * q)) & 1u) ? -(int)mag[4 * q] : (int)mag[4 * q];
			v.y = ((neg >> (4 * q + 1)) & 1u) ? -(int)mag[4 * q + 1] : (int)mag[4 * q + 1];
			v.z = ((neg >> (4 * q + 2)) & 1u) ? -(int)mag[4 * q + 2] : (int)mag[4 * q + 2];
			v.w = ((neg >> (4 * q + 3)) & 1u) ? -(int)mag[4 * q + 3] : (int)mag[4 * q + 3];
			*reinterpret_cast<Int4S *>(dst + 4 * q) = v;
		}
	} else {
#pragma unroll
		for (int i = 0; i < 16; ++i)
			if (i < nv)
				dst[i] = ((neg >> i) & 1u) ? -(int)mag[i] : (int)mag[i];
	}
}

__global__ __launch_bounds__(256) void k_tiles_init(UnpackGeom g, DWork w, int nplanes)
{
	const int tile = blockIdx.x * blockDim.x + threadIdx.x;
	const int plane = blockIdx.y;
	if (tile >= w.NT || plane >= nplanes)
		return;
	int l = 0;
	while (l + 1 < g.levels && tile >= g.tile_first[l + 1])
		++l;
	w.tile_nonsig[(long)plane * w.NT + tile] = g.tile_cnt[tile];
}

__global__ __launch_bounds__(256) void k_nch(DWork w, const unsigned long long *lens, int n)
{
	const int i = blockIdx.x * blockDim.x + threadIdx.x;
	if (i >= n)
		return;
	const unsigned long long bits = lens[i] * 8ull;
	long c = (long)((bits + CH_BITS - 1) / CH_BITS);
	c = (c + 1 + 3) / 4 * 4 - 1;
	w.nch[i] = (int)(c < w.NCH ? c : w.NCH);
}

}

template <class F> static void dwork_tables(DWork &w, unsigned *&clear_words, int C, F &&f)
{
	auto t = [&](int slot, auto *&table, long elems) { f(slot, table, elems, 1l); };
	t(SLOT_UP_SMALL, w.info, 1);
	t(SLOT_UP_SMALL, w.segidx, 48 * MAX_PLANES);
	t(SLOT_UP_SMALL, w.seg_desc, MAX_SEGS);
	t(SLOT_UP_SMALL, w.seg_symbase, MAX_SEGS);
	t(SLOT_UP_SMALL, w.seg_b2, MAX_SEGS);
	t(SLOT_UP_SMALL, w.seg_n2done, MAX_SEGS);
	t(SLOT_UP_SMALL, w.nonsig, 48);
	t(SLOT_UP_BITS, w.symbits, w.BW);
	t(SLOT_UP_TILES, w.tile_nonsig, (long)C * w.NT);
	t(SLOT_UP_TILES, w.tile_rank, (long)C * MAX_PLANES * w.NT);
	t(SLOT_UP_TILES, w.count_base, (long)C * 16);
	t(SLOT_UP_CHUNKS, w.exitX, FAM * w.NCH);
	t(SLOT_UP_CHUNKS, w.entryE, FAM * w.NCH);
	t(SLOT_UP_CHUNKS, w.cs, FAM * (w.NCH + 1));
	t(SLOT_UP_CHUNKS, w.ct, FAM * (w.NCH + 1));
	t(SLOT_UP_CHUNKS, w.cg, FAM * (w.NCH + 1));
	t(SLOT_UP_CHUNKS, w.part_s, FAM * w.NB);
	t(SLOT_UP_CHUNKS, w.part_t, FAM * w.NB);
	t(SLOT_UP_CHUNKS, w.part_g, FAM * w.NB);
	t(SLOT_UP_CHUNKS, w.hop_seg, w.MAX_HOPS);
	t(SLOT_UP_CHUNKS, w.hop_first, w.MAX_HOPS);
	t(SLOT_UP_CHUNKS, w.hop_last, w.MAX_HOPS);
	t(SLOT_UP_CHUNKS, w.hop_q0, w.MAX_HOPS);
	t(SLOT_UP_CHUNKS, w.hop_entry, w.MAX_HOPS);
	t(SLOT_UP_CHUNKS, w.hop_ntok, w.MAX_HOPS);
	t(SLOT_UP_CHUNKS, w.breaks, FAM * w.NCH);
	t(SLOT_UP_CHUNKS, w.todo[0], FAM * 64 * w.todo_cap);
	t(SLOT_UP_CHUNKS, w.todo[1], FAM * 64 * w.todo_cap);
	f(SLOT_UP_CHUNKS, w.todo_count, (long)FAM * LINK_SHARDS, (long)LINK_ROUNDS + 2);
	t(SLOT_UP_CHUNKS, w.nhops, 1);
	t(SLOT_UP_CHUNKS, w.nch, 1);
	t(SLOT_UP_CHUNKS, clear_words, 1);
	t(SLOT_UP_CHUNKS, w.idx, MAX_SEGS);
	t(SLOT_UP_CHUNKS, w.segres, MAX_SEGS);
	t(SLOT_UP_CHUNKS, w.idx_nsegs, 1);
	t(SLOT_UP_CHUNKS, w.seg_slot, MAX_SEGS + 1);
}

static void dwork_sizes(DWork &w, const UnpackGeom &g, int NT, size_t stream_stride, int n)
{
	w.NT = NT;
	w.streak_max = WALK_STREAK_MAX;
	w.scans_base = WALK_SCANS_BASE;
	w.BW = ((long)((((unsigned long long)g.total + 32ull * g.levels) * g.C * MAX_PLANES) >> 4) + 128 + 3) & ~3l;
	w.NCH = (long)((stream_stride * 8 + CH_BITS - 1) / CH_BITS);
	w.NCH = (w.NCH + 1 + 3) / 4 * 4 - 1;
	w.NB = (w.NCH + 1 + SCAN_BLOCK - 1) / SCAN_BLOCK;
	w.MAX_HOPS = 8 * MAX_SEGS + w.NCH / 8;
	w.fam = 1;
	w.todo_cap = ((w.NCH + 256) / 256 + 63) / 64 * 256 + 256;
	w.todo_round = (long)n * FAM * LINK_SHARDS;
}

#ifdef DWTX_DEBUG_HOOKS
static void debug_hooks(DWork &w, int &link_rounds)
{
	w.dbg = (unsigned long long *)getenv("DWTX_DBG_PTR") ? (unsigned long long *)strtoull(getenv("DWTX_DBG_PTR"), 0, 0) : nullptr;
	if (getenv("DWTX_DBG_STREAK"))
		w.streak_max = (unsigned)strtoul(getenv("DWTX_DBG_STREAK"), 0, 0);
	if (getenv("DWTX_DBG_SCANS"))
		w.scans_base = (unsigned)strtoul(getenv("DWTX_DBG_SCANS"), 0, 0);
	if (getenv("DWTX_DBG_ROUNDS") && atoi(getenv("DWTX_DBG_ROUNDS")) >= 1 && atoi(getenv("DWTX_DBG_ROUNDS")) <= LINK_ROUNDS)
		link_rounds = atoi(getenv("DWTX_DBG_ROUNDS"));
}
#endif

namespace {

struct DecPart {
	int first, count;
	hipStream_t stream;
	bool indexed;
	unsigned fused;
};

struct DecodeCall {
	dwtx_ctx *ctx;
	int n;
	const uint8_t *streams;
	size_t stream_stride;
	const unsigned long long *dev_lens;
	int32_t *lin, *pyr;
	dwtx_p16 p16;
	dwtx_decode_info *host_info;
	UnpackGeom g;
	DWork w;
	unsigned *clear_words;
	unsigned sq_all;
	int link_rounds;
	int fam0;
	const dwtx_index *ix_in;
	dwtx_index *ix_out;
	std::vector<int> index_segs;

	char *carve_slot(int slot)
	{
		return carve(ctx, slot, [&](Carve &c) {
			dwork_tables(w, clear_words, g.C, [&](int in_slot, auto *&table, long elems, long rows) {
				if (in_slot == slot)
					c.take(table, (size_t)n * rows * elems);
			});
		});
	}

	int queue_clears()
	{
		hipStream_t s = ctx->stream;
		const int nplanes = n * g.C;
		DWTX_HIP(hipMemsetAsync(w.todo_count, 0, sizeof(unsigned) * (LINK_ROUNDS + 2) * (size_t)w.todo_round, s));
		DWTX_HIP(hipMemsetAsync(w.nhops, 0, sizeof(int) * (size_t)n, s));
		DWTX_HIP(hipMemsetAsync(w.info, 0, (char *)w.seg_desc - (char *)w.info, s));
		const int rc = dwtx_need_part_streams(ctx, 2);
		if (rc)
			return rc;
		hipStream_t side = dwtx_part_stream(ctx, 1);
		DWTX_HIP(hipEventRecord(ctx->dec_ev.start, s));
		DWTX_HIP(hipStreamWaitEvent(side, ctx->dec_ev.start, 0));
		hipLaunchKernelGGL(k_peek, dim3(dwtx_cdiv(n, 64)), dim3(64), 0, side, g, streams, (long)stream_stride, dev_lens, w.BW, clear_words, n);
		hipLaunchKernelGGL(k_clear_bitmaps, dim3(64, n), dim3(256), 0, side, w.symbits, w.BW, clear_words);
		hipLaunchKernelGGL(k_tiles_init, dim3(dwtx_cdiv(w.NT, 256), nplanes), dim3(256), 0, side, g, w, nplanes);
		DWTX_HIP(hipEventRecord(ctx->dec_ev.cleared, side));
		DWTX_HIP(hipMemset2DAsync(lin, sizeof(int) * (size_t)g.lin_stride, 0, sizeof(int) * (size_t)g.pixels[0], nplanes, s));
		hipLaunchKernelGGL(k_nch, dim3(dwtx_cdiv(n, 256)), dim3(256), 0, s, w, dev_lens, n);
		return DWTX_OK;
	}

	DWork slice(int first) const
	{
		DWork h = w;
		unsigned *cw = clear_words;
		dwork_tables(h, cw, g.C, [&](int, auto *&table, long elems, long) { table += (size_t)first * elems; });
#ifdef DWTX_DEBUG_HOOKS
		if (h.dbg)
			h.dbg += (size_t)first * 8;
#endif
		return h;
	}

	int chunk_tables(hipStream_t st, int first, int count, int fam)
	{
		DWork h = slice(first);
		h.fam = fam;
		const unsigned char *str = streams + (size_t)first * stream_stride;
		const unsigned fblocks = (unsigned)((w.NCH + 1 + 256 * LINK_RUN - 1) / (256 * LINK_RUN));
		hipLaunchKernelGGL(k_link_first, dim3(fblocks < CHUNK_GRID ? fblocks : CHUNK_GRID, count * h.fam), dim3(256), 0, st, h, str,
			(long)stream_stride);
		int cur = 1;
		for (int r = 2; r <= link_rounds; ++r) {
			hipLaunchKernelGGL(k_link_work, dim3(LINK_SHARDS * (r <= 3 ? 4 : 1), count * h.fam), dim3(256), 0, st, h, str, (long)stream_stride, cur, r);
			cur ^= 1;
		}
		const unsigned sblocks = (unsigned)(w.NB < SCAN_GRID ? w.NB : SCAN_GRID);
		hipLaunchKernelGGL(k_scan_local, dim3(sblocks, count * h.fam), dim3(256), 0, st, h);
		hipLaunchKernelGGL(k_scan_parts, dim3(count * h.fam), dim3(256), 0, st, h);
		hipLaunchKernelGGL(k_scan_add, dim3(sblocks, count * h.fam), dim3(256), 0, st, h);
		DWTX_LAUNCH_CHECK();
		return DWTX_OK;
	}

	bool index_usable(int first, int count) const
	{
		if (!ix_in || g.levels_max < g.levels || ctx->opt[DWTX_OPT_NO_INDEX])
			return false;
		for (int i = first; i < first + count; ++i)
			if (ix_in[i].magic != DWTX_INDEX_MAGIC || ix_in[i].W != g.W || ix_in[i].H != g.H || ix_in[i].C != g.C || ix_in[i].nsegs <= 0 ||
				ix_in[i].nsegs > MAX_SEGS)
				return false;
		return true;
	}

	int walk(hipStream_t st, int first, int count, int fam, bool use_index)
	{
		DWork h = slice(first);
		h.fam = fam;
		const unsigned char *str = streams + (size_t)first * stream_stride;
		int32_t *out = lin + (size_t)first * g.C * g.lin_stride;
		DWTX_HIP(hipStreamWaitEvent(st, ctx->dec_ev.cleared, 0));
		if (use_index) {
			int maxk = 0;
			for (int i = 0; i < count; ++i) {
				const int k = ix_in[first + i].nsegs;
				index_segs[(size_t)(first + i)] = k;
				maxk = k > maxk ? k : maxk;
				DWTX_HIP(hipMemcpyAsync(h.idx + (size_t)i * MAX_SEGS, ix_in[first + i].seg, sizeof(SegIndex) * (size_t)k, hipMemcpyHostToDevice, st));
			}
			DWTX_HIP(hipMemcpyAsync(h.idx_nsegs, index_segs.data() + first, sizeof(int) * (size_t)count, hipMemcpyHostToDevice, st));
			hipLaunchKernelGGL(k_segprep, dim3(dwtx_cdiv(count, 64)), dim3(64), 0, st, h, dev_lens + first, (long)stream_stride, count);
			hipLaunchKernelGGL(k_tokenize<true>, dim3(maxk, count), dim3(64), 0, st, g, h, str, (long)stream_stride, dev_lens + first, out, count);
			hipLaunchKernelGGL(k_segjoin, dim3(count), dim3(64), 0, st, g, h, str, (long)stream_stride, dev_lens + first, out, count);
		} else
			hipLaunchKernelGGL(k_tokenize<false>, dim3(count), dim3(64), 0, st, g, h, str, (long)stream_stride, dev_lens + first, out, count);
		const unsigned hblocks = (unsigned)((w.NCH + 255) / 256);
		hipLaunchKernelGGL(k_hopbits, dim3(hblocks < CHUNK_GRID ? hblocks : CHUNK_GRID, count), dim3(256), 0, st, h, str, (long)stream_stride);
		DWTX_LAUNCH_CHECK();
		return DWTX_OK;
	}

	int fetch_infos(hipStream_t st, int first, int count)
	{
		DWTX_HIP(hipMemcpyAsync(host_info + first, w.info + first, sizeof(DecInfo) * (size_t)count, hipMemcpyDeviceToHost, st));
		DWTX_HIP(hipStreamSynchronize(st));
		return DWTX_OK;
	}

	bool gave_up(int first, int count) const
	{
		bool any = false;
		for (int i = first; i < first + count; ++i)
			any = any || host_info[i].hops == WALK_GAVE_UP;
		return any;
	}

	int walk_again(hipStream_t st, int first, int count, int fam, bool fresh_tables)
	{
		for (int i = first; i < first + count;) {
			if (host_info[i].hops != WALK_GAVE_UP) {
				++i;
				continue;
			}
			int j = i + 1;
			while (j < first + count && host_info[j].hops == WALK_GAVE_UP)
				++j;
			const int c = j - i;
			const DWork hs = slice(i);
			const long items = (long)c * FAM * LINK_SHARDS > (long)c * 48 * MAX_PLANES ? (long)c * FAM * LINK_SHARDS : (long)c * 48 * MAX_PLANES;
			hipLaunchKernelGGL(k_part_reset, dim3((unsigned)((items + 255) / 256)), dim3(256), 0, st, hs, c);
			DWTX_HIP(hipMemsetAsync(hs.symbits, 0, sizeof(unsigned) * (size_t)c * w.BW, st));
			int rc = fresh_tables ? chunk_tables(st, i, c, fam) : DWTX_OK;
			if (rc || (rc = walk(st, i, c, fam, false)))
				return rc;
			i = j;
		}
		return fetch_infos(st, first, count);
	}

	int recover(const DecPart &p)
	{
		int rc;
		if (p.indexed && gave_up(p.first, p.count)) {
			if (ctx->opt[DWTX_OPT_NO_INDEX_FALLBACK]) {
				dwtx_set_error("the sidecar index does not fit the stream (DWTX_OPT_NO_INDEX_FALLBACK forbids the serial walk)");
				return DWTX_ERR_DEVICE;
			}
			if ((rc = walk_again(p.stream, p.first, p.count, fam0, false)))
				return rc;
		}
		if (gave_up(p.first, p.count)) {
			if (ctx->opt[DWTX_OPT_NO_SECOND_WALK]) {
				dwtx_set_error("the one-family token walk gave up (DWTX_OPT_NO_SECOND_WALK forbids the second)");
				return DWTX_ERR_DEVICE;
			}
			if ((rc = walk_again(p.stream, p.first, p.count, FAM, true)))
				return rc;
		}
		return DWTX_OK;
	}

	int write_indices(int first, int count)
	{
		for (int i = first; i < first + count; ++i) {
			dwtx_index &X = ix_out[i];
			const DecInfo &D = reinterpret_cast<const DecInfo *>(host_info)[i];
			X.magic = DWTX_INDEX_MAGIC;
			X.W = g.W;
			X.H = g.H;
			X.C = g.C;
			X.reserved = 0;
			X.stream_bits = D.bits_used;
			X.nsegs = !D.status && !D.truncated && g.levels_max >= g.levels && D.nsegs > 0 && D.nsegs <= MAX_SEGS ? D.nsegs : 0;
			if (X.nsegs)
				DWTX_HIP(hipMemcpy(X.seg, w.idx + (size_t)i * MAX_SEGS, sizeof(SegIndex) * (size_t)X.nsegs, hipMemcpyDeviceToHost));
		}
		return DWTX_OK;
	}

	int scatter(DecPart &p)
	{
		const DWork h = slice(p.first);
		const int end = p.first + p.count, C = g.C;
		int pmax = 0;
		for (int i = p.first; i < end; ++i)
			if (!host_info[i].status && host_info[i].pmax > pmax)
				pmax = host_info[i].pmax;
		for (int b = pmax - 1; b >= 0; --b) {
			hipLaunchKernelGGL(k_rank, dim3(g.levels, p.count * C), dim3(1024), 0, p.stream, g, h, b);
			hipLaunchKernelGGL(k_count, dim3(dwtx_cdiv(w.NT, 256), p.count * C), dim3(256), 0, p.stream, g, h, b);
		}
		bool whole = sq_all != 0;
		for (int i = p.first; i < end; ++i)
			whole = whole && !host_info[i].status && host_info[i].level == g.levels - 1;
		UnpackGeom ga = g;
		ga.sq_levels = whole ? sq_all : 0u;
		ga.pyr = whole ? pyr + (size_t)p.first * C * g.lin_stride : nullptr;
		const bool fine = whole && p16.planes && p16.levels && !((uintptr_t)p16.planes & 15) && !(p16.levels & ~sq_all) && pmax <= 15;
		ga.fine16 = fine ? p16.planes + (size_t)p.first * C * g.lin_stride : nullptr;
		ga.lv16 = fine ? p16.levels : 0u;
		p.fused = ga.sq_levels | (fine ? DWTX_FUSED_FINE16 : 0u);
		hipLaunchKernelGGL(k_apply_all, dim3(dwtx_cdiv(w.NT, 4), p.count * C), dim3(256), 0, p.stream, ga, h,
			streams + (size_t)p.first * stream_stride, (long)stream_stride, lin + (size_t)p.first * C * g.lin_stride);
		DWTX_LAUNCH_CHECK();
		return DWTX_OK;
	}

	int run(DecPart *part, int K, int (*done)(void *user, int first, int count, unsigned fused_levels), void *user)
	{
		int rc;
		for (int k = 0; k < K; ++k) {
			DecPart &p = part[k];
			if (k > 0)
				DWTX_HIP(hipStreamWaitEvent(p.stream, ctx->dec_ev.tables[k - 1], 0));
			if ((rc = chunk_tables(p.stream, p.first, p.count, fam0)))
				return rc;
			if (k + 1 < K)
				DWTX_HIP(hipEventRecord(ctx->dec_ev.tables[k], p.stream));
			p.indexed = index_usable(p.first, p.count);
			if ((rc = walk(p.stream, p.first, p.count, fam0, p.indexed)))
				return rc;
		}
		for (int k = 0; k < K; ++k) {
			DecPart &p = part[k];
			if ((rc = fetch_infos(p.stream, p.first, p.count)) || (rc = recover(p)) || (ix_out && (rc = write_indices(p.first, p.count))) ||
				(rc = scatter(p)))
				return rc;
			if (k > 0) {
				DWTX_HIP(hipEventRecord(ctx->dec_ev.scattered[k], p.stream));
				DWTX_HIP(hipStreamWaitEvent(ctx->stream, ctx->dec_ev.scattered[k], 0));
			}
			if (done && (rc = done(user, p.first, p.count, p.fused)))
				return rc;
		}
		return DWTX_OK;
	}
};

}

int dwtx_decode_planes_ex(dwtx_ctx *ctx, int32_t *lin, int32_t *pyr, const uint8_t *streams, size_t stream_stride,
	const unsigned long long *dev_lens, int W, int H, int C, int n, int levels_max, dwtx_decode_info *host_info,
	int (*done)(void *user, int first, int count, unsigned fused_levels), void *user, dwtx_p16 p16)
{
	if (!ctx || !lin || !streams || !dev_lens || !host_info || (C != 1 && C != 3) || n < 1 || n > 65535 / 3 ||
		(stream_stride & 7) || stream_stride < 64)
		return DWTX_ERR_ARG;
	DWTX_ENTER(ctx);
	DWTX_CHECK_DIMS(W, H);
	static_assert(sizeof(dwtx_seg_index) == sizeof(SegIndex) && DWTX_INDEX_MAX_SEGS == MAX_SEGS, "SegIndex is the device image of dwtx_seg_index");
	static_assert(sizeof(dwtx_decode_info) == sizeof(DecInfo), "DecInfo is the device image of dwtx_decode_info");
	DecodeCall d{ ctx, n, streams, stream_stride, dev_lens, lin, pyr, p16, host_info };
	dwtx_tiles tiles;
	int rc = dwtx_fill_geom(ctx, W, H, C, d.g, tiles);
	if (rc)
		return rc;
	d.g.lin_stride = d.g.total;
	d.g.levels_max = levels_max < 0 || levels_max > d.g.levels ? d.g.levels : levels_max;
	d.sq_all = pyr && !((uintptr_t)pyr & 15) && !ctx->opt[DWTX_OPT_NO_SQUARE_TILES] ? dwtx_square_levels(W, H) : 0u;
	d.link_rounds = LINK_ROUNDS;
	dwork_sizes(d.w, d.g, tiles.NT, stream_stride, n);
#ifdef DWTX_DEBUG_HOOKS
	debug_hooks(d.w, d.link_rounds);
#endif
	for (int slot : { SLOT_UP_SMALL, SLOT_UP_BITS, SLOT_UP_TILES, SLOT_UP_CHUNKS })
		if (!d.carve_slot(slot))
			return DWTX_ERR_NOMEM;
	if ((rc = d.queue_clears()))
		return rc;
	d.fam0 = n <= 2 || ctx->opt[DWTX_OPT_TWO_FAMILIES] ? FAM : 1;
	d.ix_in = ctx->index_in ? ctx->index_in + ctx->index_base : nullptr;
	d.ix_out = ctx->index_out ? ctx->index_out + ctx->index_base : nullptr;
	d.index_segs.resize(d.ix_in ? (size_t)n : 0u);
	const long want_parts = ctx->opt[DWTX_OPT_DECODE_PARTS];
	const int K = n < 4 || ctx->opt[DWTX_OPT_ONE_STREAM] ? 1
		: want_parts ? (want_parts < 2 ? 2 : want_parts > DWTX_PART_STREAMS ? DWTX_PART_STREAMS : (int)want_parts) : (n >= 24 ? 4 : 2);
	if ((rc = dwtx_need_part_streams(ctx, K)))
		return rc;
	DecPart part[DWTX_PART_STREAMS];
	for (int k = 0; k < K; ++k) {
		const int first = (int)((long)n * k / K);
		part[k] = DecPart{ first, (int)((long)n * (k + 1) / K) - first, dwtx_part_stream(ctx, k), false, 0u };
	}
	rc = d.run(part, K, done, user);
	if (rc)
		for (int k = 1; k < K; ++k)
			(void)hipStreamSynchronize(part[k].stream);
	return rc;
}

extern "C" int dwtx_decode_planes(dwtx_ctx *ctx, int32_t *lin, const uint8_t *streams, size_t stream_stride,
	const unsigned long long *dev_lens, int W, int H, int C, int n, int levels_max, dwtx_decode_info *host_info)
{
	return dwtx_decode_planes_ex(ctx, lin, nullptr, streams, stream_stride, dev_lens, W, H, C, n, levels_max, host_info, nullptr, nullptr);
}
```

Before: 87170 Mpixels/s.

## Split sign bits out of the interleaved symbol bitmap into a dense sign stream

Changes the decoder's intermediate symbol bitmap from 2 bits per coefficient (one/sign interleaved) to a 1-bit significance bitmap plus a separate dense sign bitmap indexed by nonzero rank. It adds per-hop and per-segment sign bases, a sign-rank kernel, shared-memory sign windows in k_hopbits, and a reworked apply step that reads signs by rank. The aim is to halve the symbol bitmap footprint and the clearing, writing and reading traffic on it. In exchange it adds extra bookkeeping, another kernel launch, an extra bitmap to clear, and an overflow buffer for signs written by indexed segments.

```diff
diff --git a/dwt_amd/csrc/unpack.hip b/dwt_amd/csrc/unpack.hip
--- a/dwt_amd/csrc/unpack.hip
+++ b/dwt_amd/csrc/unpack.hip
@@ -14,6 +14,8 @@
 constexpr int SCAN_BLOCK = 1024;
 constexpr int LINK_ROUNDS = 12;
 constexpr int FAM = 2;
+constexpr int OWN_SIGNS = 1024;
+static_assert(MAX_SEGS <= 1024, "own_sign keeps the segment in ten bits");
 
 struct UnpackGeom {
 	int levels, C, W, H;
@@ -69,15 +71,19 @@
 	DecInfo *info;
 	int *seg_desc;
 	unsigned long long *seg_symbase;
+	unsigned long long *seg_signbase;
 	unsigned long long *seg_b2;
 	unsigned *seg_n2done;
 	int *segidx;
 	int *nonsig;
 	unsigned *symbits;
+	unsigned *signbits;
 	unsigned short *tile_nonsig;
 	unsigned *tile_rank;
+	unsigned *tile_signrank;
 	unsigned long long *count_base;
 	long BW;
+	long SW;
 	int NT;
 	unsigned short *exitX;
 	unsigned short *entryE;
@@ -88,6 +94,7 @@
 	unsigned *part_t, *part_g;
 	int *hop_seg;
 	unsigned *hop_first, *hop_last, *hop_q0;
+	unsigned *hop_t0;
 	unsigned *hop_entry;
 	unsigned *hop_ntok;
 	unsigned *breaks;
@@ -104,6 +111,9 @@
 	SegResult *segres;
 	int *idx_nsegs;
 	unsigned *seg_slot;
+	unsigned long long *own_sign;
+	unsigned *own_bits;
+	unsigned *own_count;
 	int fam;
 	unsigned streak_max, scans_base;
 };
@@ -234,26 +244,58 @@
 };
 
 struct BitmapWriter {
-	unsigned *sym;
-	long cur;
-	unsigned acc;
+	unsigned *sym, *sgn;
+	long cur, scur;
+	unsigned acc, sacc;
 	bool lead;
+	unsigned long long *own;
+	unsigned *own_bits, *own_count;
+	unsigned seg;
+	bool own_full;
 	__device__ __forceinline__ void flush()
 	{
 		if (cur >= 0 && acc && lead)
 			atomicOr(sym + cur, acc);
 		acc = 0;
 	}
+	__device__ __forceinline__ void flush_signs()
+	{
+		if (scur >= 0 && sacc) {
+			if (own) {
+				unsigned slot = 0;
+				if (lead)
+					slot = atomicAdd(own_count, 1u);
+				slot = (unsigned)__builtin_amdgcn_readfirstlane((int)slot);
+				if (slot < (unsigned)OWN_SIGNS) {
+					own[slot] = (unsigned long long)seg | (unsigned long long)scur << 10;
+					own_bits[slot] = sacc;
+				} else {
+					own_full = true;
+				}
+			} else if (lead) {
+				atomicOr(sgn + scur, sacc);
+			}
+		}
+		sacc = 0;
+	}
 	__device__ __forceinline__ void set_one(unsigned long long pos)
 	{
-		const long wi = (long)(pos >> 4);
+		const long wi = (long)(pos >> 5);
 		if (wi != cur) {
 			flush();
 			cur = wi;
 		}
-		acc |= 1u << ((pos & 15) * 2);
-	}
-	__device__ __forceinline__ void set_sign(unsigned long long pos) { acc |= 2u << ((pos & 15) * 2); }
+		acc |= 1u << (pos & 31);
+	}
+	__device__ __forceinline__ void set_sign(unsigned long long rank)
+	{
+		const long wi = (long)(rank >> 5);
+		if (wi != scur) {
+			flush_signs();
+			scur = wi;
+		}
+		sacc |= 1u << (rank & 31);
+	}
 };
 
 
@@ -877,13 +919,28 @@
 	}
 }
 
+__device__ __forceinline__ void or_bits64(unsigned *words, unsigned long long at, unsigned long long bits)
+{
+	unsigned *p = words + (at >> 5);
+	const unsigned s = (unsigned)at & 31u;
+	const unsigned long long lo = bits << s;
+	const unsigned hi = s ? (unsigned)(bits >> (64u - s)) : 0u;
+	if ((unsigned)lo)
+		atomicOr(p, (unsigned)lo);
+	if ((unsigned)(lo >> 32))
+		atomicOr(p + 1, (unsigned)(lo >> 32));
+	if (hi)
+		atomicOr(p + 2, hi);
+}
+
 __global__ __launch_bounds__(256) __attribute__((amdgpu_waves_per_eu(8))) void k_hopbits(DWork w, const unsigned char *streams, long stream_stride)
 {
 	constexpr int HB_WORDS = 16;
 	constexpr int HB_WIN = 2048;
+	constexpr int HB_SIGNS = 256 * 64 / 32 + 2;
 	__shared__ unsigned hb[256 * (HB_WORDS + 1)];
-	static_assert(HB_WIN <= 256 * (HB_WORDS + 1), "the workgroup's window lies inside the per-thread rows");
-	unsigned *win = hb;
+	static_assert(HB_WIN + HB_SIGNS <= 256 * (HB_WORDS + 1), "the workgroup's windows lie inside the per-thread rows");
+	unsigned *win = hb, *swin = hb + HB_WIN;
 	__shared__ unsigned win_last;
 	for (int i = 0; i <= HB_WORDS; ++i)
 		hb[threadIdx.x * (HB_WORDS + 1) + i] = 0u;
@@ -902,7 +959,7 @@
 		else
 			hi = mid;
 	}
-	unsigned *sym = w.symbits + img * w.BW;
+	unsigned *sym = w.symbits + img * w.BW, *sgn = w.signbits + img * w.SW;
 	const long n = w.NCH + 1;
 	ChunkWin c;
 	bool loaded = false;
@@ -917,11 +974,13 @@
 			loaded = true;
 		}
 		unsigned long long pos = w.seg_symbase[(long)img * MAX_SEGS + k] + w.hop_q0[(long)img * w.MAX_HOPS + h];
+		unsigned long long trank = w.seg_signbase[(long)img * MAX_SEGS + k] + w.hop_t0[(long)img * w.MAX_HOPS + h];
 		const unsigned entry = w.hop_entry[(long)img * w.MAX_HOPS + h];
 		unsigned left = w.hop_ntok[(long)img * w.MAX_HOPS + h];
 		int off, o;
 		if (entry == 0xffffffffu) {
 			pos += w.cs[vs * n + chunk] - w.cs[vs * n + hf[h]];
+			trank += w.ct[vs * n + chunk] - w.ct[vs * n + hf[h]];
 			const unsigned short in = w.exitX[vs * w.NCH + chunk - 1];
 			off = in & 0xff;
 			o = in >> 8;
@@ -929,17 +988,21 @@
 			off = (int)(entry & 0xff);
 			o = (int)(entry >> 8);
 		}
-		unsigned *wp = sym + (pos >> 4);
-		const unsigned rp0 = (unsigned)(pos & 15);
+		unsigned *wp = sym + (pos >> 5);
+		const unsigned rp0 = (unsigned)(pos & 31);
 		unsigned rp = rp0;
 		bool beyond = false;
+		unsigned long long sg = 0;
+		unsigned nt = 0;
 		const int off0 = off, o0 = o;
 		chunk_walk(c, off, o, [&](unsigned run, unsigned neg, bool counts) {
 			const bool take = counts && left != 0u;
 			rp += take ? run : 0u;
-			const unsigned wi = rp >> 4;
+			const unsigned wi = rp >> 5;
 			beyond = beyond || (take && wi >= (unsigned)HB_WORDS);
-			atomicOr(&mybuf[wi < (unsigned)HB_WORDS ? wi : (unsigned)HB_WORDS], take ? (1u | (neg << 1)) << ((rp & 15u) * 2u) : 0u);
+			atomicOr(&mybuf[wi < (unsigned)HB_WORDS ? wi : (unsigned)HB_WORDS], take ? 1u << (rp & 31u) : 0u);
+			sg |= (unsigned long long)(take ? neg : 0u) << (nt & 63u);
+			nt += take ? 1u : 0u;
 			rp += take ? 1u : 0u;
 			left -= take ? 1u : 0u;
 			return left != 0u || !counts;
@@ -947,18 +1010,18 @@
 		if (beyond) {
 			unsigned rq = rp0, lq = w.hop_ntok[(long)img * w.MAX_HOPS + h];
 			int off1 = off0, o1 = o0;
-			chunk_walk(c, off1, o1, [&](unsigned run, unsigned neg, bool counts) {
+			chunk_walk(c, off1, o1, [&](unsigned run, unsigned, bool counts) {
 				const bool take = counts && lq != 0u;
 				rq += take ? run : 0u;
-				if (take && (rq >> 4) >= (unsigned)HB_WORDS)
-					atomicOr(wp + (rq >> 4), (1u | (neg << 1)) << ((rq & 15u) * 2u));
+				if (take && (rq >> 5) >= (unsigned)HB_WORDS)
+					atomicOr(wp + (rq >> 5), 1u << (rq & 31u));
 				rq += take ? 1u : 0u;
 				lq -= take ? 1u : 0u;
 				return lq != 0u || !counts;
 			});
 			mybuf[HB_WORDS] = 0u;
 		}
-		const unsigned lastw = rp > rp0 ? (rp - 1) >> 4 : 0u;
+		const unsigned lastw = rp > rp0 ? (rp - 1) >> 5 : 0u;
 #pragma unroll
 		for (int i = 0; i < HB_WORDS; ++i) {
 			const unsigned v = mybuf[i];
@@ -970,6 +1033,7 @@
 				mybuf[i] = 0u;
 			}
 		}
+		or_bits64(sgn, trank, sg);
 	};
 	const bool mine = chunk < w.nch[img] && chunk >= 1;
 	if (lo < nh && hf[lo] <= first_chunk && hl[lo] >= first_chunk + blockDim.x - 1 && (lo + 1 >= nh || hf[lo + 1] > first_chunk + blockDim.x - 1)) {
@@ -985,7 +1049,12 @@
 			continue;
 		const unsigned long long seg0 = w.seg_symbase[(long)img * MAX_SEGS + k] + w.hop_q0[(long)img * w.MAX_HOPS + lo] -
 			w.cs[vs * n + hf[lo]];
-		const unsigned long long base_w = (seg0 + w.cs[vs * n + first_chunk]) >> 4;
+		const unsigned long long base_w = (seg0 + w.cs[vs * n + first_chunk]) >> 5;
+		const unsigned long long tok0 = w.seg_signbase[(long)img * MAX_SEGS + k] + w.hop_t0[(long)img * w.MAX_HOPS + lo] -
+			w.ct[vs * n + hf[lo]];
+		const unsigned ct_first = w.ct[vs * n + first_chunk];
+		const unsigned long long sbase_w = (tok0 + ct_first) >> 5;
+		const unsigned sign_bits = (unsigned)((tok0 + ct_first) & 31u) + (w.ct[vs * n + first_chunk + blockDim.x] - ct_first);
 		if (threadIdx.x == 0)
 			win_last = 0u;
 		__syncthreads();
@@ -993,25 +1062,40 @@
 			const ChunkWin cw = chunk_load((const unsigned long long *)(streams + img * stream_stride), stream_stride >> 3, chunk);
 			const unsigned short in = w.exitX[vs * w.NCH + chunk - 1];
 			int off = in & 0xff, o = in >> 8;
-			unsigned roff = (unsigned)(seg0 + w.cs[vs * n + chunk] - (base_w << 4));
+			unsigned roff = (unsigned)(seg0 + w.cs[vs * n + chunk] - (base_w << 5));
 			const unsigned roff0 = roff;
 			unsigned *gp = sym + base_w;
 			unsigned roff_prev = roff;
+			unsigned slo = 0, shi = 0, nt = 0;
 			chunk_walk_all(cw, off, o,
 				[&](unsigned run, unsigned neg, bool fits) {
 					roff += run;
-					const unsigned wi = roff >> 4;
-					const unsigned bits = fits ? (1u | (neg << 1)) << ((roff & 15u) * 2u) : 0u;
+					const unsigned wi = roff >> 5;
+					const unsigned bits = fits ? 1u << (roff & 31u) : 0u;
 					if (wi < (unsigned)HB_WIN)
 						atomicOr(&win[wi], bits);
 					else if (fits)
 						atomicOr(gp + wi, bits);
 					++roff;
+					slo = __builtin_amdgcn_alignbit(shi, slo, 1);
+					shi = __builtin_amdgcn_alignbit(neg, shi, 1);
+					++nt;
 				},
-				[&]() { roff_prev = roff; }, [&]() { roff = roff_prev; });
+				[&]() { roff_prev = roff; },
+				[&]() {
+					roff = roff_prev;
+					shi = __builtin_amdgcn_alignbit(shi, slo, 31);
+					slo <<= 1;
+					--nt;
+				});
 			if (roff > roff0) {
-				const unsigned lw = (roff - 1) >> 4;
+				const unsigned lw = (roff - 1) >> 5;
 				atomicMax(&win_last, lw < (unsigned)HB_WIN - 1u ? lw : (unsigned)HB_WIN - 1u);
+			}
+			if (nt) {
+				nt = nt < 64u ? nt : 64u;
+				const unsigned long long sg = (((unsigned long long)shi << 32) | slo) >> (64u - nt);
+				or_bits64(swin, (unsigned)(tok0 + w.ct[vs * n + chunk] - (sbase_w << 5)), sg);
 			}
 		}
 		__syncthreads();
@@ -1026,6 +1110,16 @@
 				else if (v)
 					atomicOr(gp + i, v);
 			}
+			const unsigned lasts = sign_bits ? (sign_bits - 1u) >> 5 : 0u;
+			unsigned *gs = sgn + sbase_w;
+			for (unsigned i = threadIdx.x; i <= lasts && i < (unsigned)HB_SIGNS; i += 256) {
+				const unsigned v = swin[i];
+				swin[i] = 0u;
+				if (i > 0 && i < lasts)
+					gs[i] = v;
+				else if (v)
+					atomicOr(gs + i, v);
+			}
 		}
 		__syncthreads();
 		continue;
@@ -1047,8 +1141,10 @@
 	if (t < per_round)
 		for (int r = 0; r < LINK_ROUNDS + 2; ++r)
 			h.todo_count[r * h.todo_round + t] = 0u;
-	if (t < cnt)
+	if (t < cnt) {
 		h.nhops[t] = 0;
+		h.own_count[t] = 0u;
+	}
 	if (t < (long)cnt * 48 * MAX_PLANES)
 		h.segidx[t] = 0;
 	if (t < (long)cnt * (long)(sizeof(DecInfo) / sizeof(int)))
@@ -1093,7 +1189,7 @@
 }
 
 __global__ __launch_bounds__(64) void k_peek(UnpackGeom g, const unsigned char *streams, long stream_stride, const unsigned long long *lens,
-	long BW, unsigned *clear_words, int n)
+	long BW, long SW, unsigned *clear_words, int n)
 {
 	const int img = blockIdx.x * blockDim.x + threadIdx.x;
 	if (img >= n)
@@ -1102,7 +1198,7 @@
 	const unsigned long long len = lens[img] < (unsigned long long)stream_stride ? lens[img] : (unsigned long long)stream_stride;
 	BitReader br;
 	int order, planes[3] = { 0, 0, 0 };
-	unsigned long long words = 0;
+	unsigned long long words = 0, signs = 0;
 	if (!read_preamble(br, g, s8, len, stream_stride, order, planes, nullptr, 0)) {
 		unsigned long long per = 0;
 		for (int l = 0; l < g.levels; ++l)
@@ -1110,17 +1206,23 @@
 		unsigned long long sym = ((unsigned long long)(g.pixels[1] - g.pixels[0]) + 31) & ~31ull;
 		for (int c = 0; c < g.C; ++c)
 			sym += (unsigned long long)planes[c] * per;
-		words = ((sym >> 4) + 128 + 3) & ~3ull;
-	}
-	clear_words[img] = (unsigned)(words < (unsigned long long)BW ? words : (unsigned long long)BW);
-}
-
-__global__ __launch_bounds__(256) void k_clear_bitmaps(unsigned *bits, long BW, const unsigned *clear_words)
+		words = ((sym >> 5) + 128 + 3) & ~3ull;
+		signs = (((4ull * len + 1ull + 31ull) >> 5) + 3) & ~3ull;
+	}
+	clear_words[2 * img] = (unsigned)(words < (unsigned long long)BW ? words : (unsigned long long)BW);
+	clear_words[2 * img + 1] = (unsigned)(signs < (unsigned long long)SW ? signs : (unsigned long long)SW);
+}
+
+__global__ __launch_bounds__(256) void k_clear_bitmaps(unsigned *bits, long BW, unsigned *signs, long SW, const unsigned *clear_words)
 {
 	uint4 *dst = reinterpret_cast<uint4 *>(bits + (long)blockIdx.y * BW);
-	const unsigned quads = clear_words[blockIdx.y] >> 2;
+	const unsigned quads = clear_words[2 * blockIdx.y] >> 2;
 	for (unsigned i = blockIdx.x * blockDim.x + threadIdx.x; i < quads; i += gridDim.x * blockDim.x)
 		dst[i] = make_uint4(0u, 0u, 0u, 0u);
+	uint4 *sdst = reinterpret_cast<uint4 *>(signs + (long)blockIdx.y * SW);
+	const unsigned squads = clear_words[2 * blockIdx.y + 1] >> 2;
+	for (unsigned i = blockIdx.x * blockDim.x + threadIdx.x; i < squads; i += gridDim.x * blockDim.x)
+		sdst[i] = make_uint4(0u, 0u, 0u, 0u);
 }
 
 
@@ -1241,18 +1343,26 @@
 	}
 	int *sd = w.seg_desc + (long)img * MAX_SEGS;
 	unsigned long long *ssym = w.seg_symbase + (long)img * MAX_SEGS;
+	unsigned long long *ssign = w.seg_signbase + (long)img * MAX_SEGS;
 	unsigned long long *sb2 = w.seg_b2 + (long)img * MAX_SEGS;
 	unsigned *sn2 = w.seg_n2done + (long)img * MAX_SEGS;
 	int *sidx = w.segidx + (long)img * 3 * 16 * MAX_PLANES;
 	BitmapWriter bm;
 	bm.sym = w.symbits + img * w.BW;
-	bm.cur = -1;
-	bm.acc = 0;
+	bm.sgn = w.signbits + img * w.SW;
+	bm.cur = bm.scur = -1;
+	bm.acc = bm.sacc = 0;
+	bm.own = SEG ? w.own_sign + (long)img * OWN_SIGNS : nullptr;
+	bm.own_bits = w.own_bits + (long)img * OWN_SIGNS;
+	bm.own_count = w.own_count + img;
+	bm.seg = (unsigned)seg_k;
+	bm.own_full = false;
 	bm.lead = threadIdx.x == 0;
 	const int wl = (int)threadIdx.x;
 
 	unsigned cnt = SEG ? idx[seg_k].cnt : 0u;
 	unsigned long long symtotal = SEG ? idx[seg_k].sym_base : 0ull;
+	unsigned long long signtotal = 0;
 	int nsegs = seg_k, level = -1;
 
 	const unsigned short *exitX0 = w.exitX + (long)img * FAM * w.NCH;
@@ -1280,7 +1390,7 @@
 	const long hop_cap = SEG ? (long)(w.seg_slot[(long)img * (MAX_SEGS + 1) + seg_k + 1] - w.seg_slot[(long)img * (MAX_SEGS + 1) + seg_k]) : w.MAX_HOPS;
 	int *hop_seg = w.hop_seg + hop0;
 	unsigned *hop_first = w.hop_first + hop0, *hop_last = w.hop_last + hop0, *hop_q0 = w.hop_q0 + hop0, *hop_entry = w.hop_entry + hop0,
-		*hop_ntok = w.hop_ntok + hop0;
+		*hop_ntok = w.hop_ntok + hop0, *hop_t0 = w.hop_t0 + hop0;
 
 	auto segment = [&](int c, int l, int p) -> bool {
 		const int num = g.pixels[l + 1] - g.pixels[l];
@@ -1301,6 +1411,9 @@
 		symtotal += ((unsigned long long)num + 31) & ~31ull;
 		sd[k] = c | (l << 4) | ((p + 1) << 8);
 		ssym[k] = sym0;
+		const unsigned long long sign0 = signtotal;
+		if (!SEG)
+			ssign[k] = sign0;
 		sb2[k] = 0;
 		sn2[k] = 0;
 		if (p >= 0)
@@ -1351,6 +1464,7 @@
 								hop_first[nhops] = (unsigned)ci;
 								hop_last[nhops] = (unsigned)lo;
 								hop_q0[nhops] = (unsigned)q;
+								hop_t0[nhops] = (unsigned)ones;
 								hop_entry[nhops] = 0xffffffffu;
 								hop_ntok[nhops] = 0xffffffffu;
 								++nhops;
@@ -1391,6 +1505,7 @@
 							hop_first[nhops] = (unsigned)ci;
 							hop_last[nhops] = (unsigned)ci;
 							hop_q0[nhops] = (unsigned)q;
+							hop_t0[nhops] = (unsigned)ones;
 							hop_entry[nhops] = (unsigned)rel | ((unsigned)order << 8);
 							hop_ntok[nhops] = tok;
 							++nhops;
@@ -1464,9 +1579,10 @@
 				break;
 			}
 			if (neg && p >= 0)
-				bm.set_sign(sym0 + (unsigned)q);
+				bm.set_sign(sign0 + (unsigned)(ones - 1));
 			++q;
 		}
+		signtotal += p >= 0 ? (unsigned)ones : 0u;
 		if (p >= 0) {
 			if (SEG)
 				nonsig_own[0] = n1 - ones;
@@ -1503,11 +1619,12 @@
 		const unsigned d = idx[seg_k].desc;
 		const int c = (int)(d & 15u), l = (int)((d >> 4) & 15u), p = (int)(d >> 8) - 1;
 		const unsigned long long ring = (unsigned long long)(g.pixels[l < g.levels ? l + 1 : 1] - g.pixels[l < g.levels ? l : 0]);
-		const unsigned long long sym_cap = (unsigned long long)w.BW * 16ull;
+		const unsigned long long sym_cap = (unsigned long long)w.BW * 32ull;
 		const bool sane = c < g.C && l < g.levels && p < MAX_PLANES && (unsigned long long)idx[seg_k].n1 <= ring && idx[seg_k].order <= 31u &&
 			ring + 32ull <= sym_cap && idx[seg_k].sym_base <= sym_cap - ring - 32ull;
 		const bool went = sane && segment(c, l, p);
 		bm.flush();
+		bm.flush_signs();
 		SegResult r;
 		r.bit = br.b;
 		r.order = (unsigned)order;
@@ -1516,7 +1633,7 @@
 		r.nhops = (unsigned)nhops;
 		r.hopped = hopped;
 		r.walked = walked;
-		r.ok = went && !giveup && !eof ? 1u : 0u;
+		r.ok = went && !giveup && !eof && !bm.own_full ? 1u : 0u;
 		r.pad = 0u;
 		w.segres[(long)img * MAX_SEGS + seg_k] = r;
 		return;
@@ -1526,6 +1643,7 @@
 	if (wl < 48 && (wl >> 4) < g.C && (wl & 15) < g.levels)
 		I.missing[wl] = missing_v;
 	bm.flush();
+	bm.flush_signs();
 	if (giveup) {
 		w.nhops[img] = 0;
 		I.hops = WALK_GAVE_UP;
@@ -1559,7 +1677,7 @@
 	unsigned long long at = 0;
 	for (int k = 0; good && k < K; ++k) {
 		const unsigned long long b = idx[k].bit, nb = k + 1 < K ? idx[k + 1].bit : end_bits;
-		good = b <= nb && nb <= end_bits && idx[k].sym_base < (unsigned long long)w.BW * 16ull && idx[k].order <= 31u;
+		good = b <= nb && nb <= end_bits && idx[k].sym_base < (unsigned long long)w.BW * 32ull && idx[k].order <= 31u;
 		slot[k] = (unsigned)at;
 		at += 8ull + ((nb - b) >> (CH_LOG2 + 3));
 	}
@@ -1575,6 +1693,7 @@
 	if (img >= n)
 		return;
 	const int lane = threadIdx.x;
+	__shared__ unsigned long long sbase[MAX_SEGS];
 	DecInfo &I = w.info[img];
 	info_begin(I, g);
 	const unsigned char *s8 = streams + img * stream_stride;
@@ -1602,7 +1721,7 @@
 	for (int c = 0; c < g.C; ++c)
 		for (int l = 0; l < g.levels; ++l)
 			nonsig[c * 16 + l] = g.pixels[l + 1] - g.pixels[l];
-	unsigned long long at = br.b, symtotal = 0;
+	unsigned long long at = br.b, symtotal = 0, signtotal = 0;
 	unsigned cnt = 0, hopped = 0, walked = 0;
 	int k = 0, level = -1;
 	bool good = K > 0 && g.levels_max >= g.levels;
@@ -1622,6 +1741,8 @@
 				if (p >= 0)
 					nonsig[c * 16 + l] = n1 - (int)r.ones;
 				symtotal += ((unsigned long long)num + 31) & ~31ull;
+				sbase[k] = signtotal;
+				signtotal += r.ones;
 				hopped += r.hopped;
 				walked += r.walked;
 				++k;
@@ -1629,11 +1750,24 @@
 		}
 		return good;
 	});
-	good = good && !stop && k == K;
+	good = good && !stop && k == K && w.own_count[img] <= (unsigned)OWN_SIGNS;
 	if (!good) {
 		w.nhops[img] = 0;
 		I.hops = WALK_GAVE_UP;
 		return;
+	}
+	__syncthreads();
+	for (int j = lane; j < K; j += 64)
+		w.seg_signbase[(long)img * MAX_SEGS + j] = sbase[j];
+	{
+		unsigned *sgn = w.signbits + img * w.SW;
+		const unsigned nown = w.own_count[img];
+		for (unsigned i = (unsigned)lane; i < nown; i += 64) {
+			const unsigned long long e = w.own_sign[(long)img * OWN_SIGNS + i];
+			const int j = (int)(e & 1023u);
+			if (j < K)
+				or_bits64(sgn, sbase[j] + ((e >> 10) << 5), w.own_bits[(long)img * OWN_SIGNS + i]);
+		}
 	}
 	const unsigned *slot = w.seg_slot + (long)img * (MAX_SEGS + 1);
 	const long h0 = (long)img * w.MAX_HOPS;
@@ -1644,7 +1778,7 @@
 			for (unsigned i0 = 0; i0 < nh; i0 += 64) {
 				const unsigned i = i0 + (unsigned)lane;
 				int a = 0;
-				unsigned b = 0, c2 = 0, d = 0, e = 0, f = 0;
+				unsigned b = 0, c2 = 0, d = 0, e = 0, f = 0, t0 = 0;
 				if (i < nh) {
 					a = w.hop_seg[h0 + from + i];
 					b = w.hop_first[h0 + from + i];
@@ -1652,6 +1786,7 @@
 					d = w.hop_q0[h0 + from + i];
 					e = w.hop_entry[h0 + from + i];
 					f = w.hop_ntok[h0 + from + i];
+					t0 = w.hop_t0[h0 + from + i];
 				}
 				if (i < nh) {
 					w.hop_seg[h0 + total + i] = a;
@@ -1660,6 +1795,7 @@
 					w.hop_q0[h0 + total + i] = d;
 					w.hop_entry[h0 + total + i] = e;
 					w.hop_ntok[h0 + total + i] = f;
+					w.hop_t0[h0 + total + i] = t0;
 				}
 			}
 		total += nh;
@@ -1676,28 +1812,18 @@
 }
 
 
-__global__ __launch_bounds__(1024) void k_rank(UnpackGeom g, DWork w, int p)
+template <class T>
+__device__ __forceinline__ void ring_scan(const T *in, unsigned *out, int nt)
 {
 	__shared__ unsigned wsum[16];
 	__shared__ unsigned carry;
-	const int l = blockIdx.x;
-	const int plane = blockIdx.y;
-	const int img = plane / g.C, c = plane - img * g.C;
-	const int k1 = w.info[img].status ? 0 : w.segidx[((long)img * 48 + c * 16 + l) * MAX_PLANES + p];
-	if (threadIdx.x == 0)
-		w.count_base[(long)plane * 16 + l] = k1 ? 1ull + 2ull * w.seg_symbase[(long)img * MAX_SEGS + k1 - 1] : 0ull;
-	if (!k1)
-		return;
-	const int t0 = g.tile_first[l], nt = g.tile_first[l + 1] - t0;
-	const unsigned short *ns = w.tile_nonsig + (long)plane * w.NT + t0;
-	unsigned *rank = w.tile_rank + ((long)plane * MAX_PLANES + p) * w.NT + t0;
 	const int lane = threadIdx.x & 63, wv = threadIdx.x >> 6;
 	if (threadIdx.x == 0)
 		carry = 0;
 	__syncthreads();
 	for (int b0 = 0; b0 < nt; b0 += 1024) {
 		const int i = b0 + threadIdx.x;
-		const unsigned v = i < nt ? ns[i] : 0u;
+		const unsigned v = i < nt ? in[i] : 0u;
 		unsigned inc = v;
 		for (int o = 1; o < 64; o <<= 1) {
 			const unsigned t = __shfl_up(inc, o);
@@ -1715,12 +1841,26 @@
 		}
 		const unsigned cy = carry;
 		if (i < nt)
-			rank[i] = cy + woff + inc - v;
+			out[i] = cy + woff + inc - v;
 		__syncthreads();
 		if (threadIdx.x == 0)
 			carry = cy + all;
 		__syncthreads();
 	}
+}
+
+__global__ __launch_bounds__(1024) void k_rank(UnpackGeom g, DWork w, int p)
+{
+	const int l = blockIdx.x;
+	const int plane = blockIdx.y;
+	const int img = plane / g.C, c = plane - img * g.C;
+	const int k1 = w.info[img].status ? 0 : w.segidx[((long)img * 48 + c * 16 + l) * MAX_PLANES + p];
+	if (threadIdx.x == 0)
+		w.count_base[(long)plane * 16 + l] = k1 ? 1ull + w.seg_symbase[(long)img * MAX_SEGS + k1 - 1] : 0ull;
+	if (!k1)
+		return;
+	const int t0 = g.tile_first[l], nt = g.tile_first[l + 1] - t0;
+	ring_scan(w.tile_nonsig + (long)plane * w.NT + t0, w.tile_rank + ((long)plane * MAX_PLANES + p) * w.NT + t0, nt);
 }
 
 __global__ __launch_bounds__(256) void k_count(UnpackGeom g, DWork w, int p)
@@ -1738,22 +1878,25 @@
 		return;
 	unsigned short *ns = w.tile_nonsig + (long)plane * w.NT + tile;
 	unsigned *rk = w.tile_rank + ((long)plane * MAX_PLANES + p) * w.NT + tile;
+	unsigned *sr = w.tile_signrank + ((long)plane * MAX_PLANES + p) * w.NT + tile;
 	const unsigned n = *ns;
-	if (!n)
+	if (!n) {
+		*sr = 0u;
 		return;
+	}
 	const unsigned *sym = w.symbits + img * w.BW;
-	const unsigned long long a = cb - 1ull + 2ull * *rk;
-	const unsigned long long e = a + 2ull * n;
+	const unsigned long long a = cb - 1ull + *rk;
+	const unsigned long long e = a + n;
 	const long first = (long)(a >> 5), last = (long)((e - 1) >> 5);
 	unsigned ones = 0;
-#pragma unroll 4
+#pragma unroll 3
 	for (long w0 = first & ~3l; w0 <= last; w0 += 4) {
 		const uint4 v = *reinterpret_cast<const uint4 *>(sym + w0);
 		const unsigned x[4] = { v.x, v.y, v.z, v.w };
 #pragma unroll
 		for (int q = 0; q < 4; ++q) {
 			const long wi = w0 + q;
-			unsigned m = x[q] & 0x55555555u;
+			unsigned m = x[q];
 			if (wi < first || wi > last)
 				m = 0u;
 			if (wi == first)
@@ -1763,10 +1906,24 @@
 			ones += (unsigned)__builtin_popcount(m);
 		}
 	}
+	*sr = ones;
 	if (ones) {
 		*ns = (unsigned short)(n - ones);
 		*rk |= 0x80000000u;
 	}
+}
+
+__global__ __launch_bounds__(1024) void k_signrank(UnpackGeom g, DWork w)
+{
+	const int l = blockIdx.x;
+	const int plane = blockIdx.y;
+	const int p = blockIdx.z;
+	const int img = plane / g.C, c = plane - img * g.C;
+	if (w.info[img].status || !w.segidx[((long)img * 48 + c * 16 + l) * MAX_PLANES + p])
+		return;
+	const int t0 = g.tile_first[l], nt = g.tile_first[l + 1] - t0;
+	unsigned *sr = w.tile_signrank + ((long)plane * MAX_PLANES + p) * w.NT + t0;
+	ring_scan(sr, sr, nt);
 }
 
 __device__ __forceinline__ void bit_transpose8(unsigned &lo, unsigned &hi)
@@ -1790,30 +1947,25 @@
 	unsigned char ref[16 * 16];
 };
 
+constexpr unsigned deposit4(unsigned m, unsigned b)
+{
+	unsigned out = 0, k = 0;
+	for (unsigned j = 0; j < 4; ++j)
+		if ((m >> j) & 1u) {
+			out |= ((b >> k) & 1u) << j;
+			++k;
+		}
+	return out;
+}
+
 constexpr DepositTables make_deposit_tables()
 {
 	DepositTables t{};
 	for (unsigned m = 0; m < 16; ++m) {
-		for (unsigned s = 0; s < 256; ++s) {
-			unsigned ones = 0, signs = 0, k = 0;
-			for (unsigned j = 0; j < 4; ++j)
-				if ((m >> j) & 1u) {
-					const unsigned one = (s >> (2 * k)) & 1u, sg = (s >> (2 * k + 1)) & 1u;
-					ones |= one << j;
-					signs |= (one & sg) << j;
-					++k;
-				}
-			t.sym[m * 256 + s] = (unsigned char)(ones | signs << 4);
-		}
-		for (unsigned b = 0; b < 16; ++b) {
-			unsigned out = 0, k = 0;
-			for (unsigned j = 0; j < 4; ++j)
-				if ((m >> j) & 1u) {
-					out |= ((b >> k) & 1u) << j;
-					++k;
-				}
-			t.ref[m * 16 + b] = (unsigned char)out;
-		}
+		for (unsigned sr = 0; sr < 256; ++sr)
+			t.sym[m * 256 + sr] = (unsigned char)(deposit4(m, sr >> 4) | deposit4(~m & 15u, sr & 15u) << 4);
+		for (unsigned b = 0; b < 16; ++b)
+			t.ref[m * 16 + b] = (unsigned char)deposit4(m, b);
 	}
 	return t;
 }
@@ -1850,7 +2002,7 @@
 	const int first = 16 * lane;
 	const int nv = nvalid - first < 0 ? 0 : nvalid - first > 16 ? 16 : nvalid - first;
 	const int vb = first < nvalid ? first : nvalid;
-	const unsigned *sym = w.symbits + img * w.BW;
+	const unsigned *sym = w.symbits + img * w.BW, *sgn = w.signbits + img * w.SW;
 	const unsigned *stream = (const unsigned *)(streams + img * stream_stride);
 	const long stream_words = stream_stride >> 2;
 	unsigned R[8] = { 0u, 0u, 0u, 0u, 0u, 0u, 0u, 0u };
@@ -1874,15 +2026,16 @@
 	const unsigned valid16 = nv >= 16 ? 0xffffu : (1u << nv) - 1u;
 	unsigned ins = valid16;
 
-	constexpr int AP_BATCH = 8, SYMW = 66, REFW = 34;
-	static_assert(AP_BATCH * (SYMW + REFW) <= SQ_WORDS, "the plane slices share the wave's square staging area");
+	constexpr int AP_BATCH = 8, SYMW = 34, SGNW = 34, REFW = 34;
+	static_assert(AP_BATCH * (SYMW + SGNW + REFW) <= SQ_WORDS, "the plane slices share the wave's square staging area");
 	__shared__ __attribute__((aligned(16))) unsigned ap_mem[4][SQ_WORDS];
 	unsigned (*ap_sym)[SYMW] = reinterpret_cast<unsigned (*)[SYMW]>(ap_mem[threadIdx.x >> 6]);
-	unsigned (*ap_ref)[REFW] = reinterpret_cast<unsigned (*)[REFW]>(ap_mem[threadIdx.x >> 6] + AP_BATCH * SYMW);
+	unsigned (*ap_sgn)[SGNW] = reinterpret_cast<unsigned (*)[SGNW]>(ap_mem[threadIdx.x >> 6] + AP_BATCH * SYMW);
+	unsigned (*ap_ref)[REFW] = reinterpret_cast<unsigned (*)[REFW]>(ap_mem[threadIdx.x >> 6] + AP_BATCH * (SYMW + SGNW));
 	__shared__ unsigned ap_rank[4][MAX_PLANES], ap_n2[4][MAX_PLANES], ap_refbit[4][MAX_PLANES];
 	const int wv = threadIdx.x >> 6;
 	unsigned my_tr = 0, my_n2 = 0;
-	unsigned long long my_sb = 0, my_b2 = 0;
+	unsigned long long my_sb = 0, my_b2 = 0, my_sg = 0;
 	bool my_live = false;
 	if (lane < MAX_PLANES && lane < I.planes[c]) {
 		const int k1 = w.segidx[((long)img * 48 + c * 16 + l) * MAX_PLANES + lane];
@@ -1890,6 +2043,7 @@
 			my_live = true;
 			my_tr = w.tile_rank[((long)plane * MAX_PLANES + lane) * w.NT + tile];
 			my_sb = w.seg_symbase[(long)img * MAX_SEGS + k1 - 1];
+			my_sg = w.seg_signbase[(long)img * MAX_SEGS + k1 - 1] + w.tile_signrank[((long)plane * MAX_PLANES + lane) * w.NT + tile];
 			my_b2 = w.seg_b2[(long)img * MAX_SEGS + k1 - 1];
 			my_n2 = w.seg_n2done[(long)img * MAX_SEGS + k1 - 1];
 		}
@@ -1897,6 +2051,8 @@
 	const unsigned long long livem = ballot64(my_live), flagm = ballot64(my_live && (my_tr >> 31));
 	const int ptop = flagm ? 63 - __builtin_clzll(flagm) : -1;
 	unsigned long long todo = ptop >= 0 ? livem & ((2ull << ptop) - 1ull) : 0ull;
+	const unsigned my_sgbit = (unsigned)my_sg & 31u;
+	unsigned nb = (unsigned)vb;
 	while (todo) {
 		int pl[AP_BATCH];
 		unsigned long long t2 = todo;
@@ -1905,10 +2061,10 @@
 			pl[q] = t2 ? 63 - __builtin_clzll(t2) : -1;
 			t2 &= pl[q] >= 0 ? ~(1ull << pl[q]) : ~0ull;
 		}
-		unsigned sv0[AP_BATCH], sv1[AP_BATCH], rv[AP_BATCH];
+		unsigned sv[AP_BATCH], gv[AP_BATCH], rv[AP_BATCH];
 #pragma unroll
 		for (int q = 0; q < AP_BATCH; ++q) {
-			sv0[q] = sv1[q] = rv[q] = 0u;
+			sv[q] = gv[q] = rv[q] = 0u;
 			if (pl[q] < 0)
 				continue;
 			const unsigned rank = (unsigned)__builtin_amdgcn_readlane((int)my_tr, pl[q]) & 0x7fffffffu;
@@ -1917,10 +2073,14 @@
 			const unsigned long long b2 = ((unsigned long long)(unsigned)__builtin_amdgcn_readlane((int)(my_b2 >> 32), pl[q]) << 32) |
 				(unsigned)__builtin_amdgcn_readlane((int)my_b2, pl[q]);
 			const unsigned n2 = (unsigned)__builtin_amdgcn_readlane((int)my_n2, pl[q]);
-			const unsigned *sp = sym + (sb >> 4) + (rank >> 4);
-			sv0[q] = sp[lane];
-			if (lane < SYMW - 64)
-				sv1[q] = sp[64 + lane];
+			const unsigned long long sg = ((unsigned long long)(unsigned)__builtin_amdgcn_readlane((int)(my_sg >> 32), pl[q]) << 32) |
+				(unsigned)__builtin_amdgcn_readlane((int)my_sg, pl[q]);
+			const unsigned *sp = sym + (sb >> 5) + (rank >> 5);
+			const unsigned *gp = sgn + (sg >> 5);
+			if (lane < SYMW) {
+				sv[q] = sp[lane];
+				gv[q] = gp[lane];
+			}
 			const unsigned r2t = tbase - rank;
 			const unsigned long long rbit = b2 + r2t;
 			const long rw = (long)(rbit >> 5) + lane;
@@ -1936,9 +2096,10 @@
 		for (int q = 0; q < AP_BATCH; ++q) {
 			if (pl[q] < 0)
 				continue;
-			ap_sym[q][lane] = sv0[q];
-			if (lane < SYMW - 64)
-				ap_sym[q][64 + lane] = sv1[q];
+			if (lane < SYMW) {
+				ap_sym[q][lane] = sv[q];
+				ap_sgn[q][lane] = gv[q];
+			}
 			if (lane < REFW)
 				ap_ref[q][lane] = rv[q];
 		}
@@ -1950,10 +2111,9 @@
 			todo &= ~(1ull << p);
 			const unsigned rank = ap_rank[wv][p], n2done = ap_n2[wv][p];
 			const unsigned ci = (unsigned)__builtin_popcount(ins);
-			const unsigned nb = wave_incl_add_u(ci) - ci;
-			const unsigned srel = (rank & 15u) + nb;
-			const unsigned *sw = ap_sym[q] + (srel >> 4);
-			unsigned s32 = __builtin_amdgcn_alignbit(sw[1], sw[0], (srel & 15u) * 2u);
+			const unsigned srel = (rank & 31u) + nb;
+			const unsigned *sw = ap_sym[q] + (srel >> 5);
+			unsigned s16 = __builtin_amdgcn_alignbit(sw[1], sw[0], srel & 31u);
 			const unsigned sb4 = (unsigned)vb - nb;
 			const unsigned r2 = tbase - rank + sb4;
 			const unsigned cs = (unsigned)nv - ci;
@@ -1961,17 +2121,28 @@
 			const unsigned rrel = ap_refbit[wv][p] + sb4;
 			const unsigned *rwp = ap_ref[q] + (rrel >> 5);
 			unsigned r16 = __builtin_amdgcn_alignbit(rwp[1], rwp[0], rrel & 31u) & bfm(avail, 0u);
-			const unsigned sig = valid16 & ~ins;
 			unsigned ones16 = 0, sgn16 = 0, ref16 = 0;
 #pragma unroll
 			for (int n4 = 0; n4 < 4; ++n4) {
-				const unsigned mi = (ins >> (4 * n4)) & 15u, ms = (sig >> (4 * n4)) & 15u;
-				const unsigned es = dsym[mi * 256u + (s32 & 255u)], er = dref[ms * 16u + (r16 & 15u)];
-				ones16 |= (es & 15u) << (4 * n4);
-				sgn16 |= (es >> 4) << (4 * n4);
-				ref16 |= er << (4 * n4);
-				s32 >>= 2 * __builtin_popcount(mi);
-				r16 >>= __builtin_popcount(ms);
+				const unsigned mi = (ins >> (4 * n4)) & 15u;
+				const unsigned e = dsym[mi * 256u + (s16 & 15u) * 16u + (r16 & 15u)];
+				ones16 |= (e & 15u) << (4 * n4);
+				ref16 |= (e >> 4) << (4 * n4);
+				const unsigned take = (unsigned)__builtin_popcount(mi);
+				s16 >>= take;
+				r16 >>= 4u - take;
+			}
+			const unsigned ci_next = (unsigned)__builtin_popcount(ins & ~ones16);
+			const unsigned nb_next = wave_incl_add_u(ci_next) - ci_next;
+			const unsigned grel = (unsigned)__builtin_amdgcn_readlane((int)my_sgbit, p) + (nb - nb_next);
+			nb = nb_next;
+			const unsigned *gw = ap_sgn[q] + (grel >> 5);
+			unsigned g16 = __builtin_amdgcn_alignbit(gw[1], gw[0], grel & 31u);
+#pragma unroll
+			for (int n4 = 0; n4 < 4; ++n4) {
+				const unsigned mo = (ones16 >> (4 * n4)) & 15u;
+				sgn16 |= (unsigned)dref[mo * 16u + (g16 & 15u)] << (4 * n4);
+				g16 >>= __builtin_popcount(mo);
 			}
 			const unsigned bits16 = ones16 | ref16;
 			neg |= sgn16;
@@ -2080,12 +2251,15 @@
 	t(SLOT_UP_SMALL, w.segidx, 48 * MAX_PLANES);
 	t(SLOT_UP_SMALL, w.seg_desc, MAX_SEGS);
 	t(SLOT_UP_SMALL, w.seg_symbase, MAX_SEGS);
+	t(SLOT_UP_SMALL, w.seg_signbase, MAX_SEGS);
 	t(SLOT_UP_SMALL, w.seg_b2, MAX_SEGS);
 	t(SLOT_UP_SMALL, w.seg_n2done, MAX_SEGS);
 	t(SLOT_UP_SMALL, w.nonsig, 48);
 	t(SLOT_UP_BITS, w.symbits, w.BW);
+	t(SLOT_UP_BITS, w.signbits, w.SW);
 	t(SLOT_UP_TILES, w.tile_nonsig, (long)C * w.NT);
 	t(SLOT_UP_TILES, w.tile_rank, (long)C * MAX_PLANES * w.NT);
+	t(SLOT_UP_TILES, w.tile_signrank, (long)C * MAX_PLANES * w.NT);
 	t(SLOT_UP_TILES, w.count_base, (long)C * 16);
 	t(SLOT_UP_CHUNKS, w.exitX, FAM * w.NCH);
 	t(SLOT_UP_CHUNKS, w.entryE, FAM * w.NCH);
@@ -2099,6 +2273,7 @@
 	t(SLOT_UP_CHUNKS, w.hop_first, w.MAX_HOPS);
 	t(SLOT_UP_CHUNKS, w.hop_last, w.MAX_HOPS);
 	t(SLOT_UP_CHUNKS, w.hop_q0, w.MAX_HOPS);
+	t(SLOT_UP_CHUNKS, w.hop_t0, w.MAX_HOPS);
 	t(SLOT_UP_CHUNKS, w.hop_entry, w.MAX_HOPS);
 	t(SLOT_UP_CHUNKS, w.hop_ntok, w.MAX_HOPS);
 	t(SLOT_UP_CHUNKS, w.breaks, FAM * w.NCH);
@@ -2107,11 +2282,14 @@
 	f(SLOT_UP_CHUNKS, w.todo_count, (long)FAM * LINK_SHARDS, (long)LINK_ROUNDS + 2);
 	t(SLOT_UP_CHUNKS, w.nhops, 1);
 	t(SLOT_UP_CHUNKS, w.nch, 1);
-	t(SLOT_UP_CHUNKS, clear_words, 1);
+	t(SLOT_UP_CHUNKS, clear_words, 2);
 	t(SLOT_UP_CHUNKS, w.idx, MAX_SEGS);
 	t(SLOT_UP_CHUNKS, w.segres, MAX_SEGS);
 	t(SLOT_UP_CHUNKS, w.idx_nsegs, 1);
 	t(SLOT_UP_CHUNKS, w.seg_slot, MAX_SEGS + 1);
+	t(SLOT_UP_CHUNKS, w.own_sign, OWN_SIGNS);
+	t(SLOT_UP_CHUNKS, w.own_bits, OWN_SIGNS);
+	t(SLOT_UP_CHUNKS, w.own_count, 1);
 }
 
 static void dwork_sizes(DWork &w, const UnpackGeom &g, int NT, size_t stream_stride, int n)
@@ -2119,7 +2297,8 @@
 	w.NT = NT;
 	w.streak_max = WALK_STREAK_MAX;
 	w.scans_base = WALK_SCANS_BASE;
-	w.BW = ((long)((((unsigned long long)g.total + 32ull * g.levels) * g.C * MAX_PLANES) >> 4) + 128 + 3) & ~3l;
+	w.BW = ((long)((((unsigned long long)g.total + 32ull * g.levels) * g.C * MAX_PLANES) >> 5) + 128 + 3) & ~3l;
+	w.SW = ((long)((4ull * stream_stride + 1ull + 31ull) >> 5) + 64 + 3) & ~3l;
 	w.NCH = (long)((stream_stride * 8 + CH_BITS - 1) / CH_BITS);
 	w.NCH = (w.NCH + 1 + 3) / 4 * 4 - 1;
 	w.NB = (w.NCH + 1 + SCAN_BLOCK - 1) / SCAN_BLOCK;
@@ -2186,6 +2365,7 @@
 		const int nplanes = n * g.C;
 		DWTX_HIP(hipMemsetAsync(w.todo_count, 0, sizeof(unsigned) * (LINK_ROUNDS + 2) * (size_t)w.todo_round, s));
 		DWTX_HIP(hipMemsetAsync(w.nhops, 0, sizeof(int) * (size_t)n, s));
+		DWTX_HIP(hipMemsetAsync(w.own_count, 0, sizeof(unsigned) * (size_t)n, s));
 		DWTX_HIP(hipMemsetAsync(w.info, 0, (char *)w.seg_desc - (char *)w.info, s));
 		const int rc = dwtx_need_part_streams(ctx, 2);
 		if (rc)
@@ -2193,8 +2373,8 @@
 		hipStream_t side = dwtx_part_stream(ctx, 1);
 		DWTX_HIP(hipEventRecord(ctx->dec_ev.start, s));
 		DWTX_HIP(hipStreamWaitEvent(side, ctx->dec_ev.start, 0));
-		hipLaunchKernelGGL(k_peek, dim3(dwtx_cdiv(n, 64)), dim3(64), 0, side, g, streams, (long)stream_stride, dev_lens, w.BW, clear_words, n);
-		hipLaunchKernelGGL(k_clear_bitmaps, dim3(64, n), dim3(256), 0, side, w.symbits, w.BW, clear_words);
+		hipLaunchKernelGGL(k_peek, dim3(dwtx_cdiv(n, 64)), dim3(64), 0, side, g, streams, (long)stream_stride, dev_lens, w.BW, w.SW, clear_words, n);
+		hipLaunchKernelGGL(k_clear_bitmaps, dim3(64, n), dim3(256), 0, side, w.symbits, w.BW, w.signbits, w.SW, clear_words);
 		hipLaunchKernelGGL(k_tiles_init, dim3(dwtx_cdiv(w.NT, 256), nplanes), dim3(256), 0, side, g, w, nplanes);
 		DWTX_HIP(hipEventRecord(ctx->dec_ev.cleared, side));
 		DWTX_HIP(hipMemset2DAsync(lin, sizeof(int) * (size_t)g.lin_stride, 0, sizeof(int) * (size_t)g.pixels[0], nplanes, s));
@@ -2303,6 +2483,7 @@
 			const long items = (long)c * FAM * LINK_SHARDS > (long)c * 48 * MAX_PLANES ? (long)c * FAM * LINK_SHARDS : (long)c * 48 * MAX_PLANES;
 			hipLaunchKernelGGL(k_part_reset, dim3((unsigned)((items + 255) / 256)), dim3(256), 0, st, hs, c);
 			DWTX_HIP(hipMemsetAsync(hs.symbits, 0, sizeof(unsigned) * (size_t)c * w.BW, st));
+			DWTX_HIP(hipMemsetAsync(hs.signbits, 0, sizeof(unsigned) * (size_t)c * w.SW, st));
 			int rc = fresh_tables ? chunk_tables(st, i, c, fam) : DWTX_OK;
 			if (rc || (rc = walk(st, i, c, fam, false)))
 				return rc;
@@ -2363,6 +2544,8 @@
 			hipLaunchKernelGGL(k_rank, dim3(g.levels, p.count * C), dim3(1024), 0, p.stream, g, h, b);
 			hipLaunchKernelGGL(k_count, dim3(dwtx_cdiv(w.NT, 256), p.count * C), dim3(256), 0, p.stream, g, h, b);
 		}
+		if (pmax > 0)
+			hipLaunchKernelGGL(k_signrank, dim3(g.levels, p.count * C, pmax), dim3(1024), 0, p.stream, g, h);
 		bool whole = sq_all != 0;
 		for (int i = p.first; i < end; ++i)
 			whole = whole && !host_info[i].status && host_info[i].level == g.levels - 1;
```

After: 87400 Mpixels/s, median of 6. Within noise of the previous version (+0.3%).
